# euroexa/spmv-fpga

Measured on AMD Instinct MI355X. Metric: SpMV GFLOP/s + effective HBM GB/s (% roofline), fp64, 1/2/4/8 MI355X, higher is better.
Workload: dtype f64

## Files before the change

spmv-fpga_amd/csrc/layout.cpp:

```cpp
#include <algorithm>
#include <cmath>

#include "spmv_host.hpp"

namespace spmvhw {

int plan_panels(const char *who, const IndexType *h_rp, IndexType n, uint64_t nnz, uint32_t rmax,
                const panel_options &o, panel_cut &out)
{
    const uint64_t wgs = o.wgs;
    std::vector<uint32_t> &prow = out.prow;
    double xbias = o.xbias;
    bool split_mode = false, subdivide = false;
    for (uint64_t P = o.P_first;; ++P) {
        {
            const uint64_t S = P ? wgs / P : 0;
            split_mode = !subdivide && o.allow_split && S >= 2 && P * S * 10 >= wgs * 9 &&
                         (o.force_split || 2 * S * n * o.acc_bytes * 5 <= 3 * nnz * (4 + o.val_bytes));
        }
        if (!split_mode && P > 1 && P % wgs)
            P = (P + wgs - 1) / wgs * wgs;
        P = std::min<uint64_t>(P, std::max<uint64_t>(n, 1));
        prow.assign(1, 0);
        bool ok = true;
        IndexType r = 0;
        for (uint64_t q = 1; q <= P && ok; ++q) {
            const uint64_t target =
                split_mode || xbias == 0.0
                    ? nnz * q / P
                    : (uint64_t)(double(nnz) * (double(q) - xbias * double(q & 1)) / (double(P) - xbias * double(P & 1)));
            IndexType e = (q == P) ? n : (IndexType)(std::lower_bound(h_rp, h_rp + n + 1, (IndexType)target) - h_rp);
            e = std::max(e, r);
            if (e - r > rmax && xbias != 0.0 && !split_mode && q < P)
                e = r + rmax;
            if (e - r > rmax && subdivide)
                for (; e - r > rmax; r += rmax)
                    prow.push_back(r + rmax);
            if (e - r > rmax)
                ok = false;
            prow.push_back(e);
            r = e;
        }
        if (ok)
            break;
        if (xbias != 0.0 && !split_mode) {
            xbias = 0.0;
            --P;
            continue;
        }
        if (P >= n || P > 8 * std::max<uint64_t>(min_panels(n, rmax), wgs)) {
            if (subdivide) {
                set_error(std::string(who) + ": cannot form panels");
                return 1;
            }
            subdivide = true;
            xbias = 0.0;
            P = o.P_first - 1;
        }
    }
    out.split_mode = split_mode;
    out.xbias = xbias;
    return 0;
}

static void cut_units(const std::vector<uint32_t> &poff, const std::vector<uint32_t> &punit, double d,
                      std::vector<uint32_t> &uent)
{
    const uint32_t P = (uint32_t)punit.size() - 1, U = punit[P];
    uent.assign((size_t)U + 1, 0);
    auto wc = [&](uint32_t u) { return double(u) - d * double(u & 1); };
    for (uint32_t q = 0; q < P; ++q) {
        const uint64_t chunks = (uint64_t(poff[q + 1]) - poff[q]) / kSweepChunk;
        const uint32_t k = punit[q + 1] - punit[q], u0 = punit[q];
        for (uint32_t t = 0; t < k; ++t) {
            const uint64_t c = d != 0.0 ? (uint64_t)(double(chunks) * (wc(u0 + t) - wc(u0)) / (wc(u0 + k) - wc(u0)))
                                        : chunks * t / k;
            uent[u0 + t] = (uint32_t)(poff[q] + kSweepChunk * c);
        }
    }
    uent[U] = poff[P];
}

int plan_sweep_units(const char *who, const IndexType *h_rp, const std::vector<uint32_t> &prow, bool split_mode,
                     uint64_t wgs, int pieces_override, double xbias_split, sweep_units &out)
{
    const uint32_t P = (uint32_t)(prow.size() - 1);
    std::vector<uint32_t> &off = out.off, &poff = out.poff, &punit = out.punit, &upanel = out.upanel;
    off.assign((size_t)P + 1, 0);
    poff.assign((size_t)P + 1, 0);
    out.rmax_used = 0;
    uint64_t padded = 0;
    for (uint32_t q = 0; q < P; ++q) {
        const uint64_t cnt = uint64_t(h_rp[prow[q + 1]]) - h_rp[prow[q]];
        padded += (cnt + kSweepChunk - 1) / kSweepChunk * kSweepChunk;
        off[q + 1] = (uint32_t)(off[q] + cnt);
        poff[q + 1] = (uint32_t)padded;
        out.rmax_used = std::max(out.rmax_used, prow[q + 1] - prow[q]);
    }
    if (padded > 0xFFFFFFFFull) {
        set_error(std::string(who) + ": padded entry count exceeds 32 bits");
        return 2;
    }
    uint32_t split = split_mode ? std::max<uint32_t>(1, (uint32_t)(wgs / P)) : 1;
    if (split_mode && pieces_override > 0)
        split = (uint32_t)pieces_override;
    const double mean = P ? double(padded) / P : 0.0;
    punit.assign((size_t)P + 1, 0);
    for (uint32_t q = 0; q < P; ++q) {
        const uint64_t chunks = (uint64_t(poff[q + 1]) - poff[q]) / kSweepChunk;
        uint64_t k = split * std::max<uint64_t>(
                                 1, (uint64_t)std::ceil(double(poff[q + 1] - poff[q]) / std::max(2.0 * mean, 1.0)));
        k = std::max<uint64_t>(1, std::min<uint64_t>(k, chunks));
        punit[q + 1] = punit[q] + (uint32_t)k;
    }
    upanel.assign(std::max<uint32_t>(punit[P], 1), 0);
    bool multi = false;
    for (uint32_t q = 0; q < P; ++q) {
        multi |= punit[q + 1] - punit[q] > 1;
        for (uint32_t u = punit[q]; u < punit[q + 1]; ++u)
            upanel[u] = q;
    }
    out.xbias_split = split_mode ? xbias_split : 0.0;
    cut_units(poff, punit, out.xbias_split, out.uent);
    out.sweep_split = multi ? std::max<uint32_t>(split, 2) : 1;
    return 0;
}

bin_windows plan_bin_windows(uint64_t ncols, uint64_t cus, double d)
{
    constexpr uint64_t PER = kBinPer;
    bin_windows w;
    const uint64_t wmax = w.wmax = std::min<uint64_t>((kSweepLdsBytes - 256) / sizeof(ValueType) / PER * PER, 65536);
    uint64_t &nwin = w.nwin, &W = w.W, &W0 = w.W0, &W1 = w.W1;
    if (ncols) {
        const uint64_t rounds = std::max<uint64_t>(1, (ncols + cus * wmax - 1) / (cus * wmax));
        nwin = std::min<uint64_t>(cus * rounds, (ncols + PER - 1) / PER);
        W = ((ncols + nwin - 1) / nwin + PER - 1) / PER * PER;
        nwin = (ncols + W - 1) / W;
    }
    W0 = W1 = W;
    if (!(d > -0.25 && d < 0.25) || nwin < cus || nwin % cus)
        d = 0.0;
    const uint64_t w0 = std::min<uint64_t>(wmax, (uint64_t(std::llround(W * (1.0 + d))) + PER / 2) / PER * PER);
    if (d != 0.0 && w0 >= PER && w0 < 2 * W) {
        W0 = w0;
        W1 = 2 * W - w0;
        if (W1 > wmax) {
            W0 = W1 = W;
        }
        const uint64_t pw = W0 + W1, k = ncols / pw, rem = ncols - k * pw;
        nwin = 2 * k + (rem == 0 ? 0 : rem <= W0 ? 1 : 2);
    }
    return w;
}

void plan_bin_units(const std::vector<uint32_t> &cnt, const std::vector<uint32_t> &esc, uint64_t nwin, uint64_t P,
                    uint64_t cus, bin_units &out)
{
    constexpr uint64_t PER = kBinPer;
    const uint64_t nseg = nwin * P;
    std::vector<uint64_t> &seg = out.seg, &ub = out.ub;
    seg.assign(nseg + 1, 0);
    for (uint64_t k = 0; k < nseg; ++k) {
        seg[k + 1] = seg[k] + (uint64_t(cnt[k]) + esc[k] + PER - 1) / PER * PER;
        if ((k + 1) % P == 0)
            seg[k + 1] = (seg[k + 1] + kBinAlign - 1) / kBinAlign * kBinAlign;
    }
    const uint64_t ent_pad = seg[nseg];
    ub.assign(1, 0);
    out.uwin.clear();
    const double mean = nwin ? double(ent_pad) / double(nwin) : 0.0;
    const uint64_t fill = nwin < cus ? (cus + nwin - 1) / nwin : 1;
    for (uint64_t w = 0; w < nwin; ++w) {
        const uint64_t a = seg[w * P], b = seg[(w + 1) * P], e = b - a;
        if (!e)
            continue;
        uint64_t k = std::max<uint64_t>(fill, (uint64_t)std::ceil(double(e) / std::max(2.0 * mean, 1.0)));
        k = std::max<uint64_t>(1, std::min<uint64_t>(k, e / kBinAlign));
        ub.back() = a;
        for (uint64_t t = 1; t <= k; ++t) {
            ub.push_back(a + (e / kBinAlign) * t / k * kBinAlign);
            out.uwin.push_back((uint32_t)w);
        }
    }
}

}
```

spmv-fpga_amd/csrc/plan.cpp:

```cpp
#include <algorithm>
#include <chrono>
#include <cstdlib>
#include <cstring>
#include <memory>
#include <mutex>
#include <thread>

#include "spmv_internal.hpp"

static int run_impl(spmv_plan *p, const ValueType *d_x, ValueType *d_y, hipStream_t s, bool timing);

namespace spmvhw {

int upload_staged(void *dst, const void *src, size_t bytes, hipStream_t s)
{
    constexpr size_t kChunk = 32u << 20;
    if (bytes < (4u << 20)) {
        SPMV_TRY(hipMemcpyAsync(dst, src, bytes, hipMemcpyHostToDevice, s));
        SPMV_TRY(hipStreamSynchronize(s));
        return 0;
    }
    static std::mutex mu;
    static void *buf[2] = {nullptr, nullptr};
    static hipEvent_t done[2] = {nullptr, nullptr};
    std::lock_guard<std::mutex> lk(mu);
    for (int i = 0; i < 2; ++i) {
        if (!buf[i])
            SPMV_TRY(hipHostMalloc(&buf[i], kChunk, hipHostMallocPortable));
        if (!done[i])
            SPMV_TRY(hipEventCreateWithFlags(&done[i], hipEventDisableTiming));
    }
    bool pending[2] = {false, false};
    const unsigned hc = std::thread::hardware_concurrency();
    const int T = (int)std::min(4u, hc ? hc : 1u);
    int i = 0;
    for (size_t off = 0; off < bytes; off += kChunk, i ^= 1) {
        const size_t n = std::min(kChunk, bytes - off);
        if (pending[i])
            SPMV_TRY(hipEventSynchronize(done[i]));
        auto part = [&](int t) {
            const size_t b = n * t / T, e = n * (t + 1) / T;
            std::memcpy((char *)buf[i] + b, (const char *)src + off + b, e - b);
        };
        std::vector<std::thread> th;
        for (int t = 1; t < T; ++t)
            th.emplace_back(part, t);
        part(0);
        for (auto &t : th)
            t.join();
        SPMV_TRY(hipMemcpyAsync((char *)dst + off, buf[i], n, hipMemcpyHostToDevice, s));
        SPMV_TRY(hipEventRecord(done[i], s));
        pending[i] = true;
    }
    SPMV_TRY(hipStreamSynchronize(s));
    return 0;
}

int slice_from_device(const char *who, csr_slice &out, const void *handle, int device, IndexType n, IndexType m,
                      IndexType nr_nzeros, const IndexType *d_row_ptr, const IndexType *d_col, const ValueType *d_val,
                      hipStream_t stream)
{
    if (slice_device_args(who, handle, n, d_row_ptr))
        return 1;
    SPMV_TRY(hipSetDevice(device));
    out.n = n;
    out.m = m;
    out.rp.assign(size_t(n) + 1, 0u);
    if (n) {
        SPMV_TRY(hipMemcpyAsync(out.rp.data(), d_row_ptr, out.rp.size() * sizeof(IndexType), hipMemcpyDeviceToHost,
                                stream));
        SPMV_TRY(hipStreamSynchronize(stream));
    }
    out.col = d_col;
    out.val = d_val;
    out.on_device = true;
    out.stream = stream;
    return slice_rebase(who, out, &nr_nzeros);
}

int slice_entries_on_device(const csr_slice &sl, device_scratch &up_col, device_scratch &up_val,
                            const IndexType **d_col, const ValueType **d_val)
{
    *d_col = sl.col;
    *d_val = sl.val;
    const uint64_t nnz = sl.nnz();
    if (sl.on_device || !nnz)
        return 0;
    hipStream_t s = (hipStream_t)sl.stream;
    SPMV_TRY(hipMalloc(&up_col.p, nnz * sizeof(IndexType)));
    SPMV_TRY(hipMalloc(&up_val.p, nnz * sizeof(ValueType)));
    if (upload_staged(up_col.p, sl.col, nnz * sizeof(IndexType), s) ||
        upload_staged(up_val.p, sl.val, nnz * sizeof(ValueType), s))
        return 1;
    *d_col = (const IndexType *)up_col.p;
    *d_val = (const ValueType *)up_val.p;
    return 0;
}

struct PhaseTrace {
    const bool on = std::getenv("SPMV_HW_TRACE") != nullptr;
    std::chrono::steady_clock::time_point t0 = std::chrono::steady_clock::now(), last = t0;
    void operator()(const char *phase, hipStream_t s)
    {
        if (!on)
            return;
        (void)hipStreamSynchronize(s);
        const auto now = std::chrono::steady_clock::now();
        std::fprintf(stderr, "spmv_hw trace: %-28s %9.3f ms (total %9.3f ms)\n", phase,
                     std::chrono::duration<double, std::milli>(now - last).count(),
                     std::chrono::duration<double, std::milli>(now - t0).count());
        last = now;
    }
};

constexpr int kKernelTune = -2;

static int requested_kernel()
{
    const char *e = std::getenv("SPMV_HW_KERNEL");
    if (!e || !*e || !std::strcmp(e, "auto"))
        return -1;
    if (!std::strcmp(e, "tune"))
        return kKernelTune;
    if (!std::strcmp(e, "tiles"))
        return kKernelTiles;
    if (!std::strcmp(e, "sweep"))
        return kKernelSweep;
    if (!std::strcmp(e, "gold"))
        return kKernelGold;
    if (!std::strcmp(e, "fpga"))
        return kKernelFpga;
    if (!std::strcmp(e, "blocked"))
        return kKernelBlocked;
    if (!std::strcmp(e, "slices"))
        return kKernelSlices;
    if (!std::strcmp(e, "binned"))
        return kKernelBinned;
    return -1;
}

static int build_gold(spmv_plan &p, const IndexType *h_row_ptr, const IndexType *d_col_src,
                      const ValueType *d_val_src, hipStream_t s)
{
    p.nlong = 0;
    for (IndexType r = 0; r < p.nr_rows; ++r)
        p.nlong += h_row_ptr[r + 1] - h_row_ptr[r] > (IndexType)kGoldLong;
    SPMV_TRY(hipMalloc((void **)&p.d_rp, (size_t(p.nr_rows) + 1) * sizeof(uint32_t)));
    SPMV_TRY(hipMalloc((void **)&p.d_col, std::max<uint64_t>(p.nnz, 1) * sizeof(uint32_t)));
    SPMV_TRY(hipMalloc((void **)&p.d_val, std::max<uint64_t>(p.nnz, 1) * sizeof(ValueType)));
    SPMV_TRY(hipMemcpyAsync(p.d_rp, h_row_ptr, (size_t(p.nr_rows) + 1) * sizeof(uint32_t), hipMemcpyHostToDevice, s));
    if (p.nnz) {
        SPMV_TRY(hipMemcpyAsync(p.d_col, d_col_src, p.nnz * sizeof(uint32_t), hipMemcpyDeviceToDevice, s));
        SPMV_TRY(hipMemcpyAsync(p.d_val, d_val_src, p.nnz * sizeof(ValueType), hipMemcpyDeviceToDevice, s));
    }
    SPMV_TRY(hipStreamSynchronize(s));
    return 0;
}

static int build_tiles(spmv_plan &p, const IndexType *h_row_ptr, const IndexType *d_col_src,
                       const ValueType *d_val_src, hipStream_t s)
{
    const IndexType nr_rows = p.nr_rows;
    const uint64_t nnz = p.nnz;
    p.nnz_pad = (nnz + kTileNnz - 1) / kTileNnz * kTileNnz;
    p.ntiles = p.nnz_pad / kTileNnz;

    std::vector<uint32_t> rowend(p.nnz_pad / 32, 0u);
    std::vector<uint32_t> row_id;
    if (p.has_empty)
        row_id.reserve(p.nzr);
    for (IndexType r = 0; r < nr_rows; ++r) {
        if (h_row_ptr[r + 1] > h_row_ptr[r]) {
            const uint64_t e = h_row_ptr[r + 1] - 1ull;
            rowend[e >> 5] |= 1u << (e & 31);
            if (p.has_empty)
                row_id.push_back(r);
        }
    }
    std::vector<uint32_t> tile_info(p.ntiles + 1, 0u);
    {
        uint64_t rr = 0, c = 0;
        for (uint64_t t = 0; t <= p.ntiles; ++t) {
            const uint64_t k = t * kTileNnz;
            while (rr < nr_rows && h_row_ptr[rr + 1] <= k) {
                if (h_row_ptr[rr + 1] > h_row_ptr[rr])
                    ++c;
                ++rr;
            }
            if (c > 0x7FFFFFFFull) {
                set_error("too many non-empty rows for the tile table");
                return 1;
            }
            const bool cont = k > 0 && k < nnz && !((rowend[(k - 1) >> 5] >> ((k - 1) & 31)) & 1u);
            tile_info[t] = (uint32_t)(c << 1) | (cont ? 1u : 0u);
        }
    }
    std::vector<uint32_t> cross;
    {
        auto bit = [&](uint64_t k) { return (rowend[k >> 5] >> (k & 31)) & 1u; };
        std::vector<uint8_t> has_tail(p.ntiles, 0), has_end(p.ntiles, 0);
        for (uint64_t t = 0; t < p.ntiles; ++t) {
            const uint64_t w0 = t * (kTileNnz / 32);
            for (uint64_t w = 0; w < kTileNnz / 32; ++w)
                has_end[t] |= rowend[w0 + w] != 0;
            const uint64_t last = (t + 1) * kTileNnz - 1;
            has_tail[t] = (last + 1 < nnz) && !bit(last);
        }
        for (uint64_t t = 0; t < p.ntiles; ++t) {
            if (!has_tail[t] || !(has_end[t] || t == 0 || !has_tail[t - 1]))
                continue;
            uint64_t j = t + 1;
            while (j < p.ntiles && !has_end[j])
                ++j;
            if (j >= p.ntiles) {
                set_error("internal: unterminated row crossing");
                return 1;
            }
            cross.push_back(tile_info[t + 1] >> 1);
            cross.push_back((uint32_t)t);
            cross.push_back((uint32_t)j);
        }
        p.ncross = cross.size() / 3;
    }
    auto alloc = [&](void **ptr, size_t bytes) -> hipError_t {
        *ptr = nullptr;
        return bytes ? hipMalloc(ptr, bytes) : hipSuccess;
    };
    SPMV_TRY(alloc((void **)&p.d_col, p.nnz_pad * sizeof(uint32_t)));
    SPMV_TRY(alloc((void **)&p.d_val, p.nnz_pad * sizeof(ValueType)));
    SPMV_TRY(alloc((void **)&p.d_rowend, rowend.size() * sizeof(uint32_t)));
    SPMV_TRY(alloc((void **)&p.d_tile_info, tile_info.size() * sizeof(uint32_t)));
    SPMV_TRY(alloc((void **)&p.d_head, p.ntiles * sizeof(ValueType)));
    SPMV_TRY(alloc((void **)&p.d_tail, p.ntiles * sizeof(ValueType)));
    SPMV_TRY(alloc((void **)&p.d_cross, cross.size() * sizeof(uint32_t)));
    if (p.has_empty)
        SPMV_TRY(alloc((void **)&p.d_row_id, row_id.size() * sizeof(uint32_t)));
    if (!rowend.empty())
        SPMV_TRY(hipMemcpyAsync(p.d_rowend, rowend.data(), rowend.size() * 4, hipMemcpyHostToDevice, s));
    SPMV_TRY(hipMemcpyAsync(p.d_tile_info, tile_info.data(), tile_info.size() * 4, hipMemcpyHostToDevice, s));
    if (p.has_empty && !row_id.empty())
        SPMV_TRY(hipMemcpyAsync(p.d_row_id, row_id.data(), row_id.size() * 4, hipMemcpyHostToDevice, s));
    if (!cross.empty())
        SPMV_TRY(hipMemcpyAsync(p.d_cross, cross.data(), cross.size() * 4, hipMemcpyHostToDevice, s));
    if (p.nnz_pad)
        SPMV_TRY(launch_pack(d_col_src, d_val_src, nnz, p.nnz_pad, p.nr_cols, p.d_col, p.d_val, nullptr, s));
    if (const char *xe = ablation_env("SPMV_TILE_XCD"))
        p.tile_xcd = xe[0] == '1';
    const char *nenv = ablation_env("SPMV_TILE_NARROW");
    const int narrow_min = !nenv || !*nenv ? 1 : std::atoi(nenv) == 16 ? 2 : std::atoi(nenv) == 0 ? 4 : 1;
    if (p.ntiles && narrow_min < 4) {
        uint32_t *d_span = nullptr;
        SPMV_TRY(alloc((void **)&p.d_tile_cbase, p.ntiles * sizeof(uint32_t)));
        SPMV_TRY(alloc((void **)&d_span, sizeof(uint32_t)));
        uint32_t span = 0xFFFFFFFFu;
        hipError_t e = hipMemsetAsync(d_span, 0, sizeof(uint32_t), s);
        if (e == hipSuccess)
            e = launch_tile_span(p.d_col, nnz, p.ntiles, p.d_tile_cbase, d_span, s);
        if (e == hipSuccess)
            e = hipMemcpyAsync(&span, d_span, sizeof(uint32_t), hipMemcpyDeviceToHost, s);
        if (e == hipSuccess)
            e = hipStreamSynchronize(s);
        (void)hipFree(d_span);
        SPMV_TRY(e);
        const int cb = span < 256u && narrow_min <= 1 ? 1 : span < 65536u ? 2 : 4;
        if (cb < 4) {
            SPMV_TRY(alloc(&p.d_colnar, p.nnz_pad * cb));
            SPMV_TRY(launch_narrow(p.d_col, nnz, p.nnz_pad, p.d_tile_cbase, p.d_colnar, cb, s));
            SPMV_TRY(hipStreamSynchronize(s));
            SPMV_TRY(hipFree(p.d_col));
            p.d_col = nullptr;
            p.tile_col_bytes = cb;
        } else {
            SPMV_TRY(hipFree(p.d_tile_cbase));
            p.d_tile_cbase = nullptr;
            const char *cenv = ablation_env("SPMV_TILE_CLUSTER");
            if (!(cenv && cenv[0] == '0')) {
                uint32_t *d_bad = nullptr;
                SPMV_TRY(alloc((void **)&p.d_tile_cbase, p.ntiles * 4 * sizeof(uint32_t)));
                SPMV_TRY(alloc((void **)&d_bad, sizeof(uint32_t)));
                uint32_t bad = 1;
                e = hipMemsetAsync(d_bad, 0, sizeof(uint32_t), s);
                if (e == hipSuccess)
                    e = launch_tile_clusters(p.d_col, nnz, p.ntiles, p.d_tile_cbase, d_bad, s);
                if (e == hipSuccess)
                    e = hipMemcpyAsync(&bad, d_bad, sizeof(uint32_t), hipMemcpyDeviceToHost, s);
                if (e == hipSuccess)
                    e = hipStreamSynchronize(s);
                (void)hipFree(d_bad);
                SPMV_TRY(e);
                if (!bad) {
                    SPMV_TRY(alloc(&p.d_colnar, p.nnz_pad * 2));
                    SPMV_TRY(launch_cluster_encode(p.d_col, nnz, p.nnz_pad, p.d_tile_cbase, (uint16_t *)p.d_colnar, s));
                    SPMV_TRY(hipStreamSynchronize(s));
                    SPMV_TRY(hipFree(p.d_col));
                    p.d_col = nullptr;
                    p.tile_col_bytes = 2;
                    p.tile_clustered = true;
                } else {
                    SPMV_TRY(hipFree(p.d_tile_cbase));
                    p.d_tile_cbase = nullptr;
                }
            }
        }
    }
    SPMV_TRY(hipStreamSynchronize(s));
    return 0;
}

static int fpga_params(spmv_plan &p)
{
    if (const char *v = std::getenv("SPMV_FPGA_VF")) {
        const int vf = std::atoi(v);
        if (vf != 1 && vf != 2 && vf != 4 && vf != 8) {
            set_error("SPMV_FPGA_VF must be 1, 2, 4 or 8");
            return 1;
        }
        p.fpga_vf = vf;
    }
    if (const char *b = std::getenv("SPMV_FPGA_BLOCK")) {
        const long w = std::atol(b);
        if (w < 1 || w > 0x7FFFFFFFL) {
            set_error("SPMV_FPGA_BLOCK must be a positive column count");
            return 1;
        }
        p.fpga_width = (uint32_t)w;
    }
    return 0;
}

static int order_rows_by_block(spmv_plan &p, const IndexType *h_row_ptr, hipStream_t s)
{
    if (fpga_params(p))
        return 1;
    if (!p.nnz)
        return 0;
    std::vector<uint32_t> col(p.nnz);
    SPMV_TRY(hipMemcpyAsync(col.data(), p.d_col, p.nnz * 4, hipMemcpyDeviceToHost, s));
    SPMV_TRY(hipStreamSynchronize(s));
    bool sorted = true;
    for (IndexType r = 0; r < p.nr_rows && sorted; ++r)
        for (uint64_t k = uint64_t(h_row_ptr[r]) + 1; k < h_row_ptr[r + 1]; ++k)
            if (col[k] / p.fpga_width < col[k - 1] / p.fpga_width) {
                sorted = false;
                break;
            }
    if (sorted)
        return 0;
    std::vector<ValueType> val(p.nnz);
    SPMV_TRY(hipMemcpyAsync(val.data(), p.d_val, p.nnz * sizeof(ValueType), hipMemcpyDeviceToHost, s));
    SPMV_TRY(hipStreamSynchronize(s));
    std::vector<uint32_t> idx;
    std::vector<uint32_t> c2(col);
    std::vector<ValueType> v2(val);
    for (IndexType r = 0; r < p.nr_rows; ++r) {
        const uint64_t b = h_row_ptr[r], e = h_row_ptr[r + 1];
        idx.resize(e - b);
        for (uint64_t k = b; k < e; ++k)
            idx[k - b] = (uint32_t)k;
        std::stable_sort(idx.begin(), idx.end(),
                         [&](uint32_t i, uint32_t j) { return col[i] / p.fpga_width < col[j] / p.fpga_width; });
        for (uint64_t k = b; k < e; ++k) {
            c2[k] = col[idx[k - b]];
            v2[k] = val[idx[k - b]];
        }
    }
    SPMV_TRY(hipMemcpyAsync(p.d_col, c2.data(), p.nnz * 4, hipMemcpyHostToDevice, s));
    SPMV_TRY(hipMemcpyAsync(p.d_val, v2.data(), p.nnz * sizeof(ValueType), hipMemcpyHostToDevice, s));
    SPMV_TRY(hipStreamSynchronize(s));
    return 0;
}

static int build_layout(spmv_plan &P, int kernel, bool automatic, const IndexType *h_row_ptr,
                        const IndexType *d_col, const ValueType *d_val, hipStream_t s)
{
    P.kernel = kernel;
    if (kernel == kKernelBinned) {
        const int rc = build_binned(P, h_row_ptr, d_col, d_val, s);
        if (rc == 2 && automatic) {
            P.kernel = kernel = kKernelSweep;
            (void)hipGetLastError();
        } else if (rc) {
            return 1;
        }
    }
    if (kernel == kKernelSweep || kernel == kKernelSlices) {
        const int rc = kernel == kKernelSweep ? build_sweep(P, h_row_ptr, d_col, d_val, s)
                                              : build_slices(P, h_row_ptr, d_col, d_val, s);
        if (rc == 2 && automatic)
            P.kernel = kernel = kKernelTiles;
        else if (rc)
            return 1;
    }
    if (kernel == kKernelSweep || kernel == kKernelSlices || kernel == kKernelBinned) {
    } else if (kernel == kKernelBlocked) {
        if (fpga_params(P) || build_blocked(P, h_row_ptr, d_col, d_val, s))
            return 1;
    } else if (kernel == kKernelGold || kernel == kKernelFpga) {
        if (build_gold(P, h_row_ptr, d_col, d_val, s))
            return 1;
        if (kernel == kKernelFpga && order_rows_by_block(P, h_row_ptr, s))
            return 1;
    } else {
        if (build_tiles(P, h_row_ptr, d_col, d_val, s))
            return 1;
    }
    SPMV_TRY(hipStreamSynchronize(s));
    if (P.kernel == kKernelSweep) {
        (void)launch_sweep(P, nullptr, nullptr, s, true);
    } else if (P.kernel == kKernelBinned) {
        (void)launch_binned(P, nullptr, nullptr, s, true);
    } else if (P.kernel == kKernelBlocked) {
        (void)launch_blocked(P, nullptr, nullptr, s, true);
    } else if (P.kernel == kKernelSlices) {
        (void)launch_slices(P, nullptr, nullptr, s, true);
    } else if (P.kernel == kKernelGold || P.kernel == kKernelFpga) {
        (void)launch_gold(P, nullptr, nullptr, s, true);
    } else {
        (void)launch_spmv(P, nullptr, nullptr, s, true);
        (void)launch_fixup(P, nullptr, s, true);
    }
    (void)hipGetLastError();
    return 0;
}

constexpr int kTuneSteps = 4, kTuneReps = 7;
static int time_layout(spmv_plan &P, const ValueType *d_x, ValueType *d_y, hipStream_t s, double *ms)
{
    SPMV_TRY(hipStreamSynchronize(s));
    struct Res {
        hipStream_t ts = nullptr;
        hipGraphExec_t ge = nullptr;
        hipEvent_t ev[2 * kTuneReps] = {};
        ~Res()
        {
            for (hipEvent_t e : ev)
                if (e)
                    (void)hipEventDestroy(e);
            if (ge)
                (void)hipGraphExecDestroy(ge);
            if (ts)
                (void)hipStreamDestroy(ts);
        }
    } r;
    SPMV_TRY(hipStreamCreateWithFlags(&r.ts, hipStreamNonBlocking));
    for (hipEvent_t &e : r.ev)
        SPMV_TRY(hipEventCreate(&e));
    SPMV_TRY(hipStreamBeginCapture(r.ts, hipStreamCaptureModeRelaxed));
    int rc = 0;
    for (int i = 0; i < kTuneSteps && !rc; ++i)
        rc = ::run_impl(&P, d_x, d_y, r.ts, false);
    hipGraph_t g = nullptr;
    const hipError_t ec = hipStreamEndCapture(r.ts, &g);
    if (rc) {
        if (g)
            (void)hipGraphDestroy(g);
        return rc;
    }
    SPMV_TRY(ec);
    const hipError_t ei = hipGraphInstantiate(&r.ge, g, nullptr, nullptr, 0);
    (void)hipGraphDestroy(g);
    SPMV_TRY(ei);
    SPMV_TRY(hipGraphLaunch(r.ge, r.ts));
    for (int k = 0; k < kTuneReps; ++k) {
        SPMV_TRY(hipEventRecord(r.ev[2 * k], r.ts));
        SPMV_TRY(hipGraphLaunch(r.ge, r.ts));
        SPMV_TRY(hipEventRecord(r.ev[2 * k + 1], r.ts));
    }
    SPMV_TRY(hipStreamSynchronize(r.ts));
    std::vector<double> t(kTuneReps);
    for (int k = 0; k < kTuneReps; ++k) {
        float v = 0.f;
        SPMV_TRY(hipEventElapsedTime(&v, r.ev[2 * k], r.ev[2 * k + 1]));
        t[k] = v / kTuneSteps;
    }
    std::nth_element(t.begin(), t.begin() + kTuneReps / 2, t.end());
    *ms = t[kTuneReps / 2];
    return 0;
}

int plan_create_from_slice(spmv_plan **out, int device, int op, const csr_slice &sl, int force_kernel)
{
    *out = nullptr;
    if (op == SPMV_OP_T) {
        SPMV_TRY(hipSetDevice(device));
        transposed_csr t;
        if (transpose_slice(t, sl) || plan_create_from_slice(out, device, SPMV_OP_N, t.slice, force_kernel))
            return 1;
        (*out)->op = SPMV_OP_T;
        return 0;
    }
    PhaseTrace trace;
    const IndexType nr_rows = sl.n, nr_cols = sl.m;
    const IndexType *h_row_ptr = sl.rp.data();
    hipStream_t s = (hipStream_t)sl.stream;
    const uint64_t nnz = sl.nnz();
    uint64_t nzr = 0;
    for (IndexType r = 0; r < nr_rows; ++r)
        nzr += h_row_ptr[r + 1] > h_row_ptr[r];
    if (nnz > 0 && nr_cols == 0) {
        set_error("matrix has non-zeros but zero columns");
        return 1;
    }
    SPMV_TRY(hipSetDevice(device));

    std::unique_ptr<spmv_plan> p(new spmv_plan());
    p->device = device;
    p->nr_rows = nr_rows;
    p->nr_cols = nr_cols;
    p->nnz = nnz;
    p->nzr = nzr;
    p->has_empty = nzr < nr_rows;

    device_scratch tcol, tval, trp, tbad;
    const IndexType *d_col = nullptr;
    const ValueType *d_val = nullptr;
    if (slice_entries_on_device(sl, tcol, tval, &d_col, &d_val))
        return 1;
    trace("row_ptr scan + upload", s);
    if (nnz) {
        SPMV_TRY(hipMalloc(&tbad.p, sizeof(uint32_t)));
        SPMV_TRY(hipMemsetAsync(tbad.p, 0, sizeof(uint32_t), s));
        SPMV_TRY(launch_validate(d_col, nnz, nr_cols, (uint32_t *)tbad.p, s));
        uint32_t bad = 0;
        SPMV_TRY(hipMemcpyAsync(&bad, tbad.p, sizeof(bad), hipMemcpyDeviceToHost, s));
        SPMV_TRY(hipStreamSynchronize(s));
        if (bad) {
            set_error("column index out of range (>= nr_cols)");
            return 1;
        }
    }

    const int requested = force_kernel >= 0 ? force_kernel : requested_kernel();
    int kernel = requested;
    const bool tune = kernel == kKernelTune;
    if (kernel == -1 || tune) {
        kernel = kKernelTiles;
        if (nnz && uint64_t(nr_cols) * sizeof(ValueType) >= (2ull << 20) && nnz >= 16ull * kSweepThreads) {
            SPMV_TRY(hipMalloc(&trp.p, (size_t(nr_rows) + 1) * sizeof(IndexType)));
            SPMV_TRY(hipMemcpyAsync(trp.p, h_row_ptr, (size_t(nr_rows) + 1) * sizeof(IndexType),
                                    hipMemcpyHostToDevice, s));
            if (probe_locality((const IndexType *)trp.p, d_col, nr_rows, s, &p->locality))
                return 1;
            if (p->locality < 0.3)
                kernel = kKernelSweep;
        }
        const char *det = std::getenv("SPMV_SWEEP_DETERMINISTIC");
        if (kernel == kKernelSweep && sizeof(ValueType) == 4 && nr_cols >= 5000000u && nnz >= 16000000ull &&
            !(det && det[0] == '1'))
            kernel = kKernelBinned;
    }
    const int auto_kernel = kernel;
    if (tune)
        kernel = kKernelTune;
    trace("validate + kernel choice", s);
    if (const char *t = ablation_env("SPMV_SWEEP_THREADS")) {
        const int v = std::atoi(t);
        if (v == 256 || v == 512 || v == 1024)
            p->sweep_threads = v;
    }
    auto fresh = [&]() {
        std::unique_ptr<spmv_plan> q(new spmv_plan());
        q->device = p->device;
        q->nr_rows = p->nr_rows;
        q->nr_cols = p->nr_cols;
        q->nnz = p->nnz;
        q->nzr = p->nzr;
        q->has_empty = p->has_empty;
        q->sweep_threads = p->sweep_threads;
        q->locality = p->locality;
        return q;
    };
    if (kernel == kKernelTune) {
        const char *det = std::getenv("SPMV_SWEEP_DETERMINISTIC");
        const bool fixed_bits = det && det[0] == '1';
        constexpr double kTuneBand = 0.97;
        device_scratch tx, ty;
        SPMV_TRY(hipMalloc(&tx.p, std::max<size_t>(nr_cols, 1) * sizeof(ValueType)));
        SPMV_TRY(hipMalloc(&ty.p, std::max<size_t>(nr_rows, 1) * sizeof(ValueType)));
        SPMV_TRY(hipMemsetAsync(tx.p, 0, std::max<size_t>(nr_cols, 1) * sizeof(ValueType), s));
        const int slot_of[7] = {0, -1, 1, -1, -1, 2, 3};
        std::vector<int> order = {auto_kernel};
        for (int k : {kKernelTiles, kKernelSweep, kKernelSlices, kKernelBinned})
            if (k != auto_kernel)
                order.push_back(k);
        double tuned[4] = {1e30, 1e30, 1e30, 1e30};
        std::unique_ptr<spmv_plan> kept;
        double kept_ms = 1e30;
        for (int k : order) {
            if (k == kKernelBinned && fixed_bits)
                continue;
            std::unique_ptr<spmv_plan> q = fresh();
            if (k == kKernelSlices)
                q->slice_pad_limit = 2.0;
            double t = 1e30;
            if (build_layout(*q, k, true, h_row_ptr, d_col, d_val, s) ||
                time_layout(*q, (const ValueType *)tx.p, (ValueType *)ty.p, s, &t)) {
                q.reset();
                (void)hipGetLastError();
                continue;
            }
            tuned[slot_of[k]] = t;
            if (!kept || t < kTuneBand * kept_ms) {
                kept.swap(q);
                kept_ms = t;
            }
        }
        if (!kept) {
            if (build_layout(*p, kKernelTiles, true, h_row_ptr, d_col, d_val, s))
                return 1;
        } else {
            p.swap(kept);
        }
        if (std::getenv("SPMV_HW_TRACE"))
            std::fprintf(stderr, "spmv_hw trace: tune ms tiles %.4f sweep %.4f slices %.4f binned %.4f -> kernel %d\n",
                         tuned[0], tuned[1], tuned[2], tuned[3], p->kernel);
        for (int c = 0; c < 4; ++c)
            p->tuned_ms[c] = tuned[c];
        trace("tune: build + time each", s);
    } else if (requested < 0 && kernel == kKernelTiles && nnz >= 65536) {
        std::unique_ptr<spmv_plan> r = fresh();
        r->slice_pad_limit = 1.15;
        const int rc = build_layout(*r, kKernelSlices, true, h_row_ptr, d_col, d_val, s);
        if (rc == 0 && r->kernel == kKernelSlices &&
            (r->slice_off_bytes == 2 || (r->slice_off_bytes == 1 && sizeof(ValueType) == 4)) &&
            double(r->slice_slots) * kWave <= 1.15 * double(nnz)) {
            p.swap(r);
            trace("build slice layout", s);
        } else if (rc == 0 && r->kernel == kKernelTiles) {
            r->slice_pad_limit = 0.0;
            p.swap(r);
            trace("build tile layout", s);
        } else {
            r.reset();
            (void)hipGetLastError();
            if (build_layout(*p, kKernelTiles, true, h_row_ptr, d_col, d_val, s))
                return 1;
            trace("build tile layout", s);
        }
    } else {
        if (kernel == kKernelBinned && requested < 0) {
            p->bin_skew_limit = 2.0;
            p->bin_row_limit = 0.3;
            if (const char *e = std::getenv("SPMV_BIN_ROW_LIMIT"))
                p->bin_row_limit = std::atof(e);
        }
        if (build_layout(*p, kernel, requested < 0, h_row_ptr, d_col, d_val, s))
            return 1;
        trace(p->kernel == kKernelSweep ? "build sweep layout" : p->kernel == kKernelBinned ? "build binned layout"
              : p->kernel != kKernelTiles ? "build CSR layout"
                                                                                        : "build tile layout", s);
    }
    *out = p.release();
    return 0;
}

bool product_variant(int kernel, int variant)
{
    if (variant == 0)
        return true;
    if (kernel == kKernelSweep)
        return variant == 28 || variant == kSweepTurnOrdered;
    if (kernel == kKernelBinned)
        return variant == 1 || variant == 2;
    return false;
}

}

using namespace spmvhw;

spmv_plan::~spmv_plan()
{
    (void)hipSetDevice(device);
    (void)hipDeviceSynchronize();
    for (void *ptr : {(void *)d_col, (void *)d_val, (void *)d_rowend, (void *)d_tile_info,
                      (void *)d_row_id, (void *)d_head, (void *)d_tail, (void *)d_cross, (void *)d_s_col,
                      (void *)d_s_row, (void *)d_s_val, (void *)d_panel_row, (void *)d_unit_ent, (void *)d_part, (void *)d_gcount, (void *)d_steal, (void *)d_panel_cnt, (void *)d_unit_panel, (void *)d_panel_unit, (void *)d_rp,
                      (void *)d_s_cbase, (void *)d_s_row16, (void *)d_s_d8, (void *)d_s_dbase, (void *)d_s_side, d_colnar, (void *)d_tile_cbase, (void *)d_kptr, (void *)d_kpos,
                      (void *)d_rp2, (void *)d_rl, (void *)d_chunk_row, (void *)d_bpart, (void *)d_slot_off,
                      (void *)d_sbase, (void *)d_slice_len, (void *)d_b_val, (void *)d_b_colw, (void *)d_b_rowp,
                      d_b_prod_alloc, (void *)d_b_seg, (void *)d_b_seg_hi, (void *)d_b_ub, (void *)d_b_uwin})
        if (ptr)
            (void)hipFree(ptr);
    for (void *ptr : gpart)
        (void)hipFree(ptr);
    for (hipEvent_t e : ev)
        (void)hipEventDestroy(e);
    if (gexec)
        (void)hipGraphExecDestroy(gexec);
    if (gstream)
        (void)hipStreamDestroy(gstream);
    if (gstream2)
        (void)hipStreamDestroy(gstream2);
}

uint64_t spmv_plan::device_bytes() const
{
    if (kernel == kKernelGold || kernel == kKernelFpga)
        return (uint64_t(nr_rows) + 1) * 4 + nnz * (4 + sizeof(ValueType));
    if (kernel == kKernelSlices)
        return slice_slots * kWave * (sizeof(ValueType) + slice_off_bytes) + slice_slots * (slice_clustered ? 16 : 4) +
               (nslices + 1) * 4 +
               uint64_t(nr_rows) * 4;
    if (kernel == kKernelBlocked)
        return nnz * (2 + sizeof(ValueType)) + (nkpairs + 1) * 4 + nkpairs * (4 + 2 + sizeof(ValueType)) +
               (uint64_t(nr_rows) + 1) * 4 + (nchunks + 1) * 4 + nunits * 8 + 4;
    if (kernel == kKernelBinned)
        return ent_pad * (2 * sizeof(ValueType) + 2 + (b_delta ? 1 : 2)) + (uint64_t(b_nwin) * npanels + 1) * 8 +
               (b_nunits + 1) * 12 + (npanels + 1) * 4;
    if (kernel == kKernelSweep)
        return ent_pad * ((d_s_col ? sizeof(uint32_t) : 0) + (sweep_packed ? 0 : sizeof(uint16_t)) + sizeof(ValueType)) +
               (npanels + 1) * 4 + (nunits + 1) * 4 + (sweep_packed ? ent_pad / kSweepChunk * 4 : 0) +
               (sweep_split > 1 ? nunits * (uint64_t(panel_rmax) + 1) * sweep_acc_bytes : 0) + nunits * 4 + (npanels + 1) * 4 +
               (d_panel_cnt ? npanels * 4 : 0) +
               (sweep_delta ? ent_pad * 3 + ent_pad / kSweepChunk * 4 + sweep_side_chunks * kSweepChunk * 4 : 0);
    return nnz_pad * (tile_col_bytes + sizeof(ValueType)) + nnz_pad / 8 + (ntiles + 1) * 4 +
           (tile_col_bytes < 4 ? ntiles * (tile_clustered ? 16 : 4) : 0) +
           (has_empty ? nzr * 4 : 0) + ntiles * 2 * sizeof(ValueType) + ncross * 12;
}

uint64_t spmv_plan::algorithmic_bytes() const
{
    return nnz * (sizeof(ValueType) + 4) + (uint64_t(nr_rows) + 1) * 4 +
           uint64_t(nr_cols) * sizeof(ValueType) + uint64_t(nr_rows) * sizeof(ValueType);
}

static int create_device(const char *who, spmv_plan **plan, int device, int op, IndexType nr_rows, IndexType nr_cols,
                         IndexType nr_nzeros, const IndexType *d_row_ptr, const IndexType *d_col_ind,
                         const ValueType *d_values, void *stream)
{
    csr_slice sl;
    if (slice_from_device(who, sl, plan, device, nr_rows, nr_cols, nr_nzeros, d_row_ptr, d_col_ind, d_values,
                          (hipStream_t)stream))
        return 1;
    return plan_create_from_slice(plan, device, op, sl);
}

static int create_host(const char *who, spmv_plan **plan, int device, int op, const csr_matrix *m, IndexType row_begin,
                       IndexType row_end)
{
    csr_slice sl;
    if (slice_from_host(who, sl, plan, m, row_begin, row_end))
        return 1;
    return plan_create_from_slice(plan, device, op, sl);
}

extern "C" {

int spmv_plan_create_device(spmv_plan **plan, int device, IndexType nr_rows, IndexType nr_cols,
                            IndexType nr_nzeros, const IndexType *d_row_ptr,
                            const IndexType *d_col_ind, const ValueType *d_values, void *stream)
{
    return create_device("spmv_plan_create_device", plan, device, SPMV_OP_N, nr_rows, nr_cols, nr_nzeros, d_row_ptr,
                         d_col_ind, d_values, stream);
}

int spmv_plan_create_host(spmv_plan **plan, int device, const csr_matrix *m, IndexType row_begin,
                          IndexType row_end)
{
    return create_host("spmv_plan_create_host", plan, device, SPMV_OP_N, m, row_begin, row_end);
}

int spmv_plan_create_device_op(spmv_plan **plan, int device, int op, IndexType nr_rows, IndexType nr_cols,
                               IndexType nr_nzeros, const IndexType *d_row_ptr, const IndexType *d_col_ind,
                               const ValueType *d_values, void *stream)
{
    if (bad_op("spmv_plan_create_device_op", op))
        return 1;
    return create_device(op == SPMV_OP_N ? "spmv_plan_create_device" : "spmv_plan_create_device_op", plan, device, op,
                         nr_rows, nr_cols, nr_nzeros, d_row_ptr, d_col_ind, d_values, stream);
}

int spmv_plan_create_host_op(spmv_plan **plan, int device, int op, const csr_matrix *m, IndexType row_begin,
                             IndexType row_end)
{
    if (bad_op("spmv_plan_create_host_op", op))
        return 1;
    return create_host(op == SPMV_OP_N ? "spmv_plan_create_host" : "spmv_plan_create_host_op", plan, device, op, m,
                       row_begin, row_end);
}

int spmv_plan_get_op(const spmv_plan *plan, int *op)
{
    if (!plan || !op) {
        set_error("spmv_plan_get_op: null argument");
        return 1;
    }
    *op = plan->op;
    return 0;
}

static int run_impl(spmv_plan *p, const ValueType *d_x, ValueType *d_y, hipStream_t s, bool timing)
{
    if (p->nr_rows == 0)
        return 0;
    if (p->kernel == kKernelTiles && (p->has_empty || p->nnz == 0))
        SPMV_TRY(hipMemsetAsync(d_y, 0, size_t(p->nr_rows) * sizeof(ValueType), s));
    hipEvent_t e0 = nullptr, e1 = nullptr;
    if (timing) {
        if (p->ev_used + 2 > p->ev.size()) {
            for (int i = 0; i < 2; ++i) {
                hipEvent_t e;
                SPMV_TRY(hipEventCreate(&e));
                p->ev.push_back(e);
            }
        }
        e0 = p->ev[p->ev_used];
        e1 = p->ev[p->ev_used + 1];
        p->ev_used += 2;
        SPMV_TRY(hipEventRecord(e0, s));
    }
    if (p->kernel != kKernelTiles) {
        SPMV_TRY(p->kernel == kKernelSweep     ? launch_sweep(*p, d_x, d_y, s)
                 : p->kernel == kKernelBinned  ? launch_binned(*p, d_x, d_y, s)
                 : p->kernel == kKernelBlocked ? launch_blocked(*p, d_x, d_y, s)
                 : p->kernel == kKernelSlices  ? launch_slices(*p, d_x, d_y, s)
                                               : launch_gold(*p, d_x, d_y, s));
        if (timing)
            SPMV_TRY(hipEventRecord(e1, s));
        return 0;
    }
    SPMV_TRY(launch_spmv(*p, d_x, d_y, s));
    if (timing)
        SPMV_TRY(hipEventRecord(e1, s));
    SPMV_TRY(launch_fixup(*p, d_y, s));
    return 0;
}

int spmv_plan_run(const spmv_plan *cp, const ValueType *d_x, ValueType *d_y, void *stream)
{
    if (!cp) {
        set_error("spmv_plan_run: null plan");
        return 1;
    }
    spmv_plan *p = const_cast<spmv_plan *>(cp);
    SPMV_TRY(hipSetDevice(p->device));
    return run_impl(p, d_x, d_y, (hipStream_t)stream, p->timing);
}

static bool graph_overlaps(const spmv_plan *p)
{
    return p->kernel == kKernelSweep && p->sweep_split > 1 && !p->d_panel_cnt && p->d_part &&
           !(p->sweep_variant >= 37 && p->sweep_variant <= 39);
}

static int graph_part2(spmv_plan *p)
{
    if (p->gpart.empty()) {
        void *b = nullptr;
        SPMV_TRY(hipMalloc(&b, p->nunits * (uint64_t(p->panel_rmax) + 1) * p->sweep_acc_bytes));
        p->gpart.push_back(b);
    }
    return 0;
}

static int capture_overlapped(spmv_plan *p, const ValueType *d_x, ValueType *d_y, int iters)
{
    constexpr int R = 2;
    if (graph_part2(p))
        return 1;
    if (!p->gstream2)
        SPMV_TRY(hipStreamCreateWithFlags(&p->gstream2, hipStreamNonBlocking));
    std::vector<hipEvent_t> ev(2 * size_t(iters), nullptr);
    auto destroy = [&] {
        for (hipEvent_t e : ev)
            if (e)
                (void)hipEventDestroy(e);
    };
    for (auto &e : ev)
        if (hipEventCreateWithFlags(&e, hipEventDisableTiming) != hipSuccess) {
            destroy();
            set_error("spmv_plan_run_graph: hipEventCreate failed");
            return 1;
        }
    hipStream_t a = p->gstream, b = p->gstream2;
    hipError_t e = hipStreamBeginCapture(a, hipStreamCaptureModeRelaxed);
    for (int k = 0; k < iters && e == hipSuccess; ++k) {
        void *part = k % R ? p->gpart[k % R - 1] : p->d_part;
        if (k >= R)
            e = hipStreamWaitEvent(a, ev[2 * (k - R) + 1], 0);
        if (e == hipSuccess)
            e = launch_sweep(*p, d_x, d_y, a, false, 1, part);
        if (e == hipSuccess)
            e = hipEventRecord(ev[2 * k], a);
        if (e == hipSuccess)
            e = hipStreamWaitEvent(b, ev[2 * k], 0);
        if (e == hipSuccess)
            e = launch_sweep(*p, d_x, d_y, b, false, 2, part);
        if (e == hipSuccess)
            e = hipEventRecord(ev[2 * k + 1], b);
    }
    if (e == hipSuccess)
        e = hipStreamWaitEvent(a, ev[2 * (iters - 1) + 1], 0);
    hipGraph_t g = nullptr;
    const hipError_t ec = hipStreamEndCapture(a, &g);
    destroy();
    if (e != hipSuccess || ec != hipSuccess) {
        if (g)
            (void)hipGraphDestroy(g);
        set_error(std::string("spmv_plan_run_graph: overlapped capture: ") +
                  hipGetErrorString(e != hipSuccess ? e : ec));
        return 1;
    }
    const hipError_t ei = hipGraphInstantiate(&p->gexec, g, nullptr, nullptr, 0);
    (void)hipGraphDestroy(g);
    SPMV_TRY(ei);
    return 0;
}

static int capture_behind(spmv_plan *p, const ValueType *d_x, ValueType *d_y, int iters)
{
    if (graph_part2(p))
        return 1;
    if (!p->d_gcount) {
        SPMV_TRY(hipMalloc(&p->d_gcount, 2 * sizeof(uint32_t)));
        SPMV_TRY(hipMemset(p->d_gcount, 0, 2 * sizeof(uint32_t)));
    }
    int ncu = 0;
    SPMV_TRY(hipDeviceGetAttribute(&ncu, hipDeviceAttributeMultiprocessorCount, p->device));
    auto part_of = [&](int k) { return (k & 1) ? p->gpart[0] : p->d_part; };
    hipStream_t a = p->gstream;
    hipError_t e = hipStreamBeginCapture(a, hipStreamCaptureModeRelaxed);
    for (int k = 0; k < iters && e == hipSuccess; ++k) {
        sweep_behind bh;
        bh.cpart = k ? part_of(k - 1) : nullptr;
        bh.ccount = p->d_gcount + (k & 1);
        bh.cnext = p->d_gcount + ((k + 1) & 1);
        bh.blocks = (uint32_t)std::max(ncu, 1);
        if (const char *v = ablation_env("SPMV_BEHIND_BLOCKS"))
            bh.blocks = (uint32_t)std::max(1, atoi(v));
        if (const char *v = ablation_env("SPMV_BEHIND_ROWS"))
            bh.rows_per_thread = (uint32_t)std::max(1, atoi(v) / std::max(1, p->sweep_threads));
        e = launch_sweep(*p, d_x, d_y, a, false, 1, part_of(k), &bh);
    }
    if (e == hipSuccess)
        e = launch_sweep(*p, d_x, d_y, a, false, 2, part_of(iters - 1));
    hipGraph_t g = nullptr;
    const hipError_t ec = hipStreamEndCapture(a, &g);
    if (e != hipSuccess || ec != hipSuccess) {
        if (g)
            (void)hipGraphDestroy(g);
        set_error(std::string("spmv_plan_run_graph: behind capture: ") + hipGetErrorString(e != hipSuccess ? e : ec));
        return 1;
    }
    const hipError_t ei = hipGraphInstantiate(&p->gexec, g, nullptr, nullptr, 0);
    (void)hipGraphDestroy(g);
    SPMV_TRY(ei);
    return 0;
}

static int graph_form(const spmv_plan *p)
{
    const int best = p->kernel == kKernelSweep && sweep_behind_ok(*p) ? 2 : graph_overlaps(p) ? 1 : 0;
    if (const char *f = ablation_env("SPMV_GRAPH_FORM")) {
        const std::string v(f);
        if (v == "serial")
            return 0;
        if (v == "dag" && best >= 1)
            return 1;
    }
    return best;
}

int spmv_plan_run_graph(spmv_plan *p, const ValueType *d_x, ValueType *d_y, int iters, void *stream)
{
    if (!p || iters < 1) {
        set_error("spmv_plan_run_graph: null plan or iters < 1");
        return 1;
    }
    hipStream_t s = (hipStream_t)stream;
    SPMV_TRY(hipSetDevice(p->device));
    if (!p->gexec || p->gx != d_x || p->gy != d_y || p->giters != iters) {
        if (p->gexec) {
            SPMV_TRY(hipGraphExecDestroy(p->gexec));
            p->gexec = nullptr;
        }
        if (!p->gstream)
            SPMV_TRY(hipStreamCreateWithFlags(&p->gstream, hipStreamNonBlocking));
        const int form = iters >= 2 ? graph_form(p) : 0;
        if (form == 2) {
            if (capture_behind(p, d_x, d_y, iters))
                return 1;
        } else if (form == 1) {
            if (capture_overlapped(p, d_x, d_y, iters))
                return 1;
        } else {
            SPMV_TRY(hipStreamBeginCapture(p->gstream, hipStreamCaptureModeRelaxed));
            int rc = 0;
            for (int i = 0; i < iters && !rc; ++i)
                rc = run_impl(p, d_x, d_y, p->gstream, false);
            hipGraph_t g = nullptr;
            const hipError_t ec = hipStreamEndCapture(p->gstream, &g);
            if (rc) {
                if (g)
                    (void)hipGraphDestroy(g);
                return rc;
            }
            SPMV_TRY(ec);
            const hipError_t ei = hipGraphInstantiate(&p->gexec, g, nullptr, nullptr, 0);
            (void)hipGraphDestroy(g);
            SPMV_TRY(ei);
        }
        p->gx = d_x;
        p->gy = d_y;
        p->giters = iters;
    }
    hipEvent_t e0 = nullptr, e1 = nullptr;
    if (p->timing) {
        for (int i = 0; p->ev_used + 2 > p->ev.size() && i < 2; ++i) {
            hipEvent_t e;
            SPMV_TRY(hipEventCreate(&e));
            p->ev.push_back(e);
        }
        e0 = p->ev[p->ev_used];
        e1 = p->ev[p->ev_used + 1];
        p->ev_used += 2;
        SPMV_TRY(hipEventRecord(e0, s));
    }
    SPMV_TRY(hipGraphLaunch(p->gexec, s));
    if (p->timing)
        SPMV_TRY(hipEventRecord(e1, s));
    return 0;
}

int spmv_plan_get_stats(const spmv_plan *p, spmv_plan_stats *st)
{
    if (!p || !st) {
        set_error("spmv_plan_get_stats: null argument");
        return 1;
    }
    std::memset(st, 0, sizeof(*st));
    st->nr_rows = p->nr_rows;
    st->nr_cols = p->nr_cols;
    st->nr_nzeros = p->nnz;
    st->nr_nonempty_rows = p->nzr;
    const bool csr = p->kernel == kKernelGold || p->kernel == kKernelFpga;
    st->nr_tiles = (p->kernel == kKernelSweep || p->kernel == kKernelBlocked) ? p->nunits
                   : p->kernel == kKernelBinned                               ? p->npanels
                   : p->kernel == kKernelSlices                               ? p->nslices
                   : csr                                                      ? p->nlong
                                                                              : p->ntiles;
    st->tile_nnz = p->kernel == kKernelSlices   ? p->slice_slots * kWave
                   : p->kernel == kKernelSweep  ? (p->nunits ? p->ent_pad / p->nunits : 0)
                   : p->kernel == kKernelBinned ? (p->npanels ? p->ent_pad / p->npanels : 0)
                   : p->kernel == kKernelBlocked ? (p->nunits ? p->nnz / p->nunits : 0)
                   : csr                         ? (uint64_t)kGoldLong
                                                 : kTileNnz;
    st->device_bytes = p->device_bytes();
    st->algorithmic_bytes = p->algorithmic_bytes();
    st->device = p->device;
    st->kernel = p->kernel;
    st->blocks = p->kernel == kKernelBlocked ? (uint32_t)((uint64_t(p->nr_cols) + p->fpga_width - 1) / p->fpga_width) : 1;
    st->format = (p->kernel == kKernelSlices && p->slice_off_bytes < 4 ? 1 : 0) | (p->slice_clustered ? 16 : 0) |
                 (p->kernel == kKernelSlices && p->slice_off_bytes == 1 ? 8 : 0) | (p->tile_col_bytes < 4 ? 1 : 0) | (p->sweep_packed ? 2 : 0) | (p->sweep_lane_order ? 4 : 0) | (p->sweep_delta ? 64 : 0) |
                 (p->tile_col_bytes == 1 ? 8 : 0) | (p->tile_clustered ? 16 : 0) |
                 (p->kernel == kKernelBinned && p->b_delta ? 32 : 0) |
                 (p->kernel == kKernelSweep && p->sweep_steal &&
                          (p->sweep_variant == 37 || p->sweep_variant == 38 || p->sweep_variant == 39) ? 128 : 0) |
                 (graph_form(p) == 2 ? 256 : graph_form(p) == 1 ? 512 : 0) |
                 (p->kernel == kKernelSweep && p->sweep_split > 1 && p->xbias_split > 0.0 ? 1024 : 0) |
                 (p->kernel == kKernelSweep && p->sweep_split > 1 && p->xbias_split < 0.0 ? 2048 : 0) |
                 (p->kernel == kKernelSweep && p->sweep_wide ? 4096 : 0);
    return 0;
}

int spmv_plan_set_variant(spmv_plan *p, int variant)
{
    if (!p || variant < 0 || (variant > 63 && variant != kSweepTurn && variant != kSweepTurnOrdered)) {
        set_error("spmv_plan_set_variant: bad arguments");
        return 1;
    }
#ifndef SPMV_ABLATIONS
    if (!product_variant(p->kernel, variant)) {
        set_error("spmv_plan_set_variant: measurement variant (tools library only)");
        return 1;
    }
#endif
    if (p->kernel == kKernelSweep && variant == 0)
        variant = 28;
    if (p->kernel == kKernelSweep) {
        if ((variant < 36 || variant > 39) && variant != 28 && sweep_materialize_rc(*p))
            return 1;
        p->sweep_variant = variant;
    } else if (p->kernel == kKernelBinned) {
        if (variant > 7 && !(variant >= 51 && variant <= 52)) {
            set_error("spmv_plan_set_variant: binned variants are 0-7");
            return 1;
        }
        if (p->d_b_seg_hi) {
            SPMV_TRY(hipSetDevice(p->device));
            SPMV_TRY(hipFree(p->d_b_seg_hi));
            p->d_b_seg_hi = nullptr;
            p->b_seg_base = 0;
        }
        if (variant == 1 || variant == 2) {
            SPMV_TRY(hipSetDevice(p->device));
            const uint64_t nseg = uint64_t(p->b_nwin) * p->npanels + 1;
            std::vector<uint64_t> h(nseg);
            SPMV_TRY(hipMemcpy(h.data(), p->d_b_seg, nseg * 8, hipMemcpyDeviceToHost));
            const uint64_t base = (variant == 1 ? (1ull << 31) : (1ull << 32)) - h[nseg - 1] / 2;
            for (auto &v : h)
                v += base;
            SPMV_TRY(hipMalloc((void **)&p->d_b_seg_hi, nseg * 8));
            SPMV_TRY(hipMemcpy(p->d_b_seg_hi, h.data(), nseg * 8, hipMemcpyHostToDevice));
            p->b_seg_base = base;
        }
        p->variant = variant;
    } else {
        p->variant = variant & 3;
    }
    if (p->gexec) {
        (void)hipSetDevice(p->device);
        (void)hipGraphExecDestroy(p->gexec);
        p->gexec = nullptr;
    }
    return 0;
}

int spmv_plan_set_timing(spmv_plan *p, int enable)
{
    if (!p) {
        set_error("spmv_plan_set_timing: null plan");
        return 1;
    }
    p->timing = enable != 0;
    p->ev_used = 0;
    return 0;
}

int spmv_plan_get_timing(spmv_plan *p, double *mean_ms, double *total_ms, int *launches)
{
    if (!p) {
        set_error("spmv_plan_get_timing: null plan");
        return 1;
    }
    SPMV_TRY(hipSetDevice(p->device));
    double tot = 0.0;
    int n = 0;
    for (size_t i = 0; i + 1 < p->ev_used; i += 2) {
        SPMV_TRY(hipEventSynchronize(p->ev[i + 1]));
        float ms = 0.f;
        SPMV_TRY(hipEventElapsedTime(&ms, p->ev[i], p->ev[i + 1]));
        tot += ms;
        ++n;
    }
    p->ev_used = 0;
    if (mean_ms)
        *mean_ms = n ? tot / n : 0.0;
    if (total_ms)
        *total_ms = tot;
    if (launches)
        *launches = n;
    return 0;
}

void spmv_plan_destroy(spmv_plan *p) { delete p; }

}
```

spmv-fpga_amd/csrc/spmv_host.hpp:

```cpp
#pragma once

#include <algorithm>
#include <cstddef>
#include <cstdint>
#include <cstdlib>
#include <string>
#include <vector>

#include "csr_hw_wrapper.h"

namespace spmvhw {

void set_error(const std::string &msg);
const char *get_error();

inline const char *ablation_env(const char *name)
{
#ifdef SPMV_ABLATIONS
    return std::getenv(name);
#else
    (void)name;
    return nullptr;
#endif
}

struct csr_slice {
    IndexType n = 0, m = 0;
    std::vector<IndexType> rp;
    const IndexType *col = nullptr;
    const ValueType *val = nullptr;
    bool on_device = false;
    void *stream = nullptr;
    uint64_t nnz() const { return rp.empty() ? 0 : rp.back(); }
};

int slice_from_host(const char *who, csr_slice &out, const void *handle, const csr_matrix *m, IndexType row_begin,
                    IndexType row_end);
int slice_device_args(const char *who, const void *handle, IndexType n, const IndexType *d_row_ptr);
int slice_rebase(const char *who, csr_slice &s, const IndexType *nr_nzeros = nullptr);

constexpr uint64_t kSweepLdsBytes = 160 * 1024;
constexpr uint64_t kSweepChunk = 128;
constexpr uint32_t kBinPer = 16 / sizeof(ValueType);
constexpr uint64_t kBinAlign = 128;

inline uint64_t min_panels(uint64_t n, uint32_t rmax) { return std::max<uint64_t>(1, (n + rmax - 1) / rmax); }

struct panel_options {
    uint64_t wgs = 256;
    uint64_t P_first = 1;
    bool allow_split = false;
    bool force_split = false;
    uint64_t acc_bytes = 8, val_bytes = sizeof(ValueType);
    double xbias = 0.0;
};
struct panel_cut {
    std::vector<uint32_t> prow;
    bool split_mode = false;
    double xbias = 0.0;
};
int plan_panels(const char *who, const IndexType *h_rp, IndexType n, uint64_t nnz, uint32_t rmax,
                const panel_options &o, panel_cut &out);

struct sweep_units {
    std::vector<uint32_t> off, poff;
    std::vector<uint32_t> punit;
    std::vector<uint32_t> upanel;
    std::vector<uint32_t> uent;
    uint32_t rmax_used = 0;
    uint32_t sweep_split = 1;
    double xbias_split = 0.0;
};
int plan_sweep_units(const char *who, const IndexType *h_rp, const std::vector<uint32_t> &prow, bool split_mode,
                     uint64_t wgs, int pieces_override, double xbias_split, sweep_units &out);

struct bin_windows {
    uint64_t wmax = 0, nwin = 1, W = kBinPer, W0 = kBinPer, W1 = kBinPer;
};
bin_windows plan_bin_windows(uint64_t ncols, uint64_t cus, double d);

struct bin_units {
    std::vector<uint64_t> seg;
    std::vector<uint64_t> ub;
    std::vector<uint32_t> uwin;
};
void plan_bin_units(const std::vector<uint32_t> &cnt, const std::vector<uint32_t> &esc, uint64_t nwin, uint64_t P,
                    uint64_t cus, bin_units &out);

double timestamp_us();

struct add_part {
    ValueType *dst;
    const ValueType *src;
    uint64_t count;
    void *ready;
};

struct accum_options {
    bool prefault = true;
    bool split = true;
    int threads = 16;
};

double host_accumulate(const add_part *parts, size_t nparts, int (*wait)(void *ready, std::string *err),
                       const accum_options &opts, bool *failed, std::string *err);

void prefault(ValueType *p, uint64_t count);

}
```

spmv-fpga_amd/csrc/spmv_internal.hpp:

```cpp
#pragma once

#include <hip/hip_runtime.h>
#include <cstdint>
#include <cstdio>
#include <string>
#include <vector>

#include "csr_hw_wrapper.h"
#include "spmv_host.hpp"

namespace spmvhw {

constexpr int kWave = 64;
constexpr int kLaneEntries = 4;
constexpr int kStep = kWave * kLaneEntries;
constexpr int kTileSteps = 2;
constexpr int kTileNnz = kStep * kTileSteps;
constexpr int kBlockThreads = 256;
constexpr int kSweepThreads = 1024;
constexpr int kSweepTurn = 91;
constexpr int kSweepTurnOrdered = 94;

constexpr int kKernelTiles = 0;
constexpr int kKernelGold = 1;
constexpr int kKernelSweep = 2;
constexpr int kKernelFpga = 3;
constexpr int kKernelBlocked = 4;
constexpr int kKernelSlices = 5;
constexpr int kKernelBinned = 6;
constexpr int kGoldLong = 128;

__device__ __forceinline__ uint32_t wave_inclusive_sum(uint32_t v0)
{
    uint32_t v = v0;
    v += __builtin_amdgcn_update_dpp(0u, v0, 0x111, 0xf, 0xf, true);
    v += __builtin_amdgcn_update_dpp(0u, v0, 0x112, 0xf, 0xf, true);
    v += __builtin_amdgcn_update_dpp(0u, v0, 0x113, 0xf, 0xf, true);
    v += __builtin_amdgcn_update_dpp(0u, v, 0x114, 0xf, 0xe, true);
    v += __builtin_amdgcn_update_dpp(0u, v, 0x118, 0xf, 0xc, true);
    v += __builtin_amdgcn_update_dpp(0u, v, 0x142, 0xa, 0xf, false);
    v += __builtin_amdgcn_update_dpp(0u, v, 0x143, 0xc, 0xf, false);
    return v;
}

}

struct spmv_plan {
    int device = 0;
    IndexType nr_rows = 0, nr_cols = 0;
    uint64_t nnz = 0, nnz_pad = 0;
    uint64_t nzr = 0;
    uint64_t ntiles = 0;
    bool has_empty = false;
    int kernel = 0;
    int op = SPMV_OP_N;
    int variant = 0;
    int sweep_variant = 28;

    uint32_t *d_col = nullptr;
    void *d_colnar = nullptr;
    uint32_t *d_tile_cbase = nullptr;
    int tile_col_bytes = 4;
    bool tile_clustered = false;
    bool tile_xcd = false;
    ValueType *d_val = nullptr;
    uint32_t *d_rowend = nullptr;
    uint32_t *d_tile_info = nullptr;
    uint32_t *d_row_id = nullptr;
    ValueType *d_head = nullptr;
    ValueType *d_tail = nullptr;
    uint32_t *d_cross = nullptr;
    uint64_t ncross = 0;

    uint32_t *d_rp = nullptr;
    uint64_t nlong = 0;
    int fpga_vf = 1;
    uint32_t fpga_width = 32768;

    uint32_t *d_kptr = nullptr;
    uint32_t *d_kpos = nullptr;
    uint32_t *d_rp2 = nullptr;
    uint16_t *d_rl = nullptr;
    uint32_t *d_chunk_row = nullptr;
    ValueType *d_bpart = nullptr;
    uint64_t nkpairs = 0, nchunks = 0;
    bool blocked_xlds = false;

    uint32_t *d_slot_off = nullptr;
    uint32_t *d_sbase = nullptr;
    uint32_t *d_slice_len = nullptr;
    uint64_t nslices = 0, slice_slots = 0;
    int slice_off_bytes = 4;
    bool slice_clustered = false;
    bool slice_acc_native = false;
    double slice_pad_limit = 0.0;

    uint64_t npanels = 0, ent_pad = 0;
    uint64_t nunits = 0;
    uint32_t sweep_split = 1;
    uint32_t *d_unit_panel = nullptr;
    uint32_t *d_panel_unit = nullptr;
    void *d_part = nullptr;
    std::vector<void *> gpart;
    uint32_t *d_gcount = nullptr;
    double xbias_split = 0.0;
    unsigned long long *d_steal = nullptr;
    bool sweep_steal = false;
    uint32_t *d_panel_cnt = nullptr;
    int sweep_acc_bytes = 8;
    uint32_t panel_rmax = 0;
    int sweep_threads = spmvhw::kSweepThreads;
    uint32_t *d_s_col = nullptr;
    uint16_t *d_s_row = nullptr;
    ValueType *d_s_val = nullptr;
    uint32_t *d_panel_row = nullptr;
    uint32_t *d_unit_ent = nullptr;
    uint32_t *d_s_cbase = nullptr;
    bool sweep_packed = false;
    bool sweep_lane_order = false;
    bool sweep_det = false;
    uint16_t *d_s_row16 = nullptr;
    uint8_t *d_s_d8 = nullptr;
    uint32_t *d_s_dbase = nullptr;
    uint32_t *d_s_side = nullptr;
    uint64_t sweep_side_chunks = 0;
    bool sweep_delta = false;
    bool sweep_wide = false;
    uint32_t b_nwin = 0, b_W = 0;
    uint32_t b_W1 = 0;
    uint64_t b_nunits = 0;
    ValueType *d_b_val = nullptr;
    uint16_t *d_b_colw = nullptr;
    void *d_b_rowp = nullptr;
    bool b_delta = false;
    bool b_prod_temporal = false;
    ValueType *d_b_prod = nullptr;
    void *d_b_prod_alloc = nullptr;
    uint64_t *d_b_seg = nullptr;
    uint64_t *d_b_seg_hi = nullptr;
    uint64_t b_seg_base = 0;
    uint64_t *d_b_ub = nullptr;
    uint32_t *d_b_uwin = nullptr;
    double bin_skew_limit = 0.0;
    double bin_row_limit = 0.0;
    uint32_t *y_flag = nullptr;
    uint32_t y_epoch = 0;
    ValueType *y_host = nullptr;
    double locality = -1.0;
    double tuned_ms[4] = {-1.0, -1.0, -1.0, -1.0};

    bool timing = false;
    std::vector<hipEvent_t> ev;
    size_t ev_used = 0;

    hipGraphExec_t gexec = nullptr;
    hipStream_t gstream = nullptr;
    hipStream_t gstream2 = nullptr;
    const ValueType *gx = nullptr;
    ValueType *gy = nullptr;
    int giters = 0;

    uint64_t device_bytes() const;
    uint64_t algorithmic_bytes() const;
    ~spmv_plan();
};

namespace spmvhw {

template <typename K, typename... Args>
inline void launch_or_warm(bool warm, K kernel, dim3 grid, dim3 block, size_t lds, hipStream_t s, Args... args)
{
    if (warm) {
        hipFuncAttributes a;
        (void)hipFuncGetAttributes(&a, reinterpret_cast<const void *>(kernel));
    } else {
        hipLaunchKernelGGL(kernel, grid, block, lds, s, args...);
    }
}

hipError_t launch_spmv(const spmv_plan &p, const ValueType *d_x, ValueType *d_y, hipStream_t s, bool warm = false);
hipError_t launch_fixup(const spmv_plan &p, ValueType *d_y, hipStream_t s, bool warm = false);
hipError_t launch_pack(const IndexType *d_col_src, const ValueType *d_val_src, uint64_t nnz,
                       uint64_t nnz_pad, uint32_t ncols, uint32_t *d_col, ValueType *d_val,
                       uint32_t *d_bad, hipStream_t s);
hipError_t launch_validate(const IndexType *d_col, uint64_t nnz, uint32_t ncols, uint32_t *d_bad, hipStream_t s);
hipError_t launch_tile_span(const uint32_t *d_col, uint64_t nnz, uint64_t ntiles, uint32_t *d_cbase,
                            uint32_t *d_maxspan, hipStream_t s);
hipError_t launch_tile_clusters(const uint32_t *d_col, uint64_t nnz, uint64_t ntiles, uint32_t *d_bases,
                                uint32_t *d_bad, hipStream_t s);
hipError_t launch_cluster_encode(const uint32_t *d_col, uint64_t nnz, uint64_t nnz_pad, const uint32_t *d_bases,
                                 uint16_t *d_out, hipStream_t s);
hipError_t launch_narrow(const uint32_t *d_col, uint64_t nnz, uint64_t nnz_pad, const uint32_t *d_cbase,
                         void *d_out, int bytes, hipStream_t s);

hipError_t launch_gold(const spmv_plan &p, const ValueType *d_x, ValueType *d_y, hipStream_t s, bool warm = false);

hipError_t launch_blocked(const spmv_plan &p, const ValueType *d_x, ValueType *d_y, hipStream_t s, bool warm = false);
int build_blocked(spmv_plan &p, const IndexType *h_rp, const IndexType *d_col_src, const ValueType *d_val_src,
                  hipStream_t s);

hipError_t launch_slices(const spmv_plan &p, const ValueType *d_x, ValueType *d_y, hipStream_t s, bool warm = false);
int build_slices(spmv_plan &p, const IndexType *h_rp, const IndexType *d_col_src, const ValueType *d_val_src,
                 hipStream_t s);
hipError_t launch_slices_multi(const spmv_plan &p, int nvec, const ValueType *d_X, ValueType *d_Y, hipStream_t s,
                               bool warm = false);

hipError_t launch_binned(const spmv_plan &p, const ValueType *d_x, ValueType *d_y, hipStream_t s, bool warm = false);
int build_binned(spmv_plan &p, const IndexType *h_rp, const IndexType *d_col_src, const ValueType *d_val_src,
                 hipStream_t s);

struct sweep_behind {
    const void *cpart = nullptr;
    uint32_t *ccount = nullptr;
    uint32_t *cnext = nullptr;
    uint32_t blocks = 0;
    uint32_t rows_per_thread = 4;
};
hipError_t launch_sweep(const spmv_plan &p, const ValueType *d_x, ValueType *d_y, hipStream_t s, bool warm = false,
                        int phase = 0, void *part = nullptr, const sweep_behind *behind = nullptr);
bool sweep_behind_ok(const spmv_plan &p);
bool product_variant(int kernel, int variant);
int build_sweep(spmv_plan &p, const IndexType *h_rp, const IndexType *d_col_src, const ValueType *d_val_src,
                hipStream_t s);
int probe_locality(const IndexType *d_rp, const IndexType *d_col, IndexType n, hipStream_t s, double *frac);
int sweep_materialize_rc(spmv_plan &p);
bool sweep_can_flag_panels(const spmv_plan &p);

struct device_scratch {
    void *p = nullptr;
    ~device_scratch()
    {
        if (p)
            (void)hipFree(p);
    }
};
template <typename T>
struct device_buf : device_scratch {
    device_buf() = default;
    device_buf(const device_buf &) = delete;
    T *get() const { return static_cast<T *>(p); }
    operator T *() const { return get(); }
    hipError_t alloc(uint64_t count) { return hipMalloc(&p, count * sizeof(T)); }
    hipError_t release()
    {
        void *q = p;
        p = nullptr;
        return q ? hipFree(q) : hipSuccess;
    }
    void swap(T *&owned)
    {
        T *q = get();
        p = owned;
        owned = q;
    }
};
template <typename K, typename... Args>
inline hipError_t launch_items(K kernel, uint64_t items, unsigned block, hipStream_t s, Args... args)
{
    hipLaunchKernelGGL(kernel, dim3((unsigned)((items + block - 1) / block)), dim3(block), 0, s, args...);
    return hipGetLastError();
}
inline int device_cu_count(int device)
{
    hipDeviceProp_t prop;
    return hipGetDeviceProperties(&prop, device) == hipSuccess && prop.multiProcessorCount > 0
               ? prop.multiProcessorCount
               : 256;
}

int upload_staged(void *dst, const void *src, size_t bytes, hipStream_t s);
int slice_from_device(const char *who, csr_slice &out, const void *handle, int device, IndexType n, IndexType m,
                      IndexType nr_nzeros, const IndexType *d_row_ptr, const IndexType *d_col, const ValueType *d_val,
                      hipStream_t stream);
int slice_entries_on_device(const csr_slice &sl, device_scratch &up_col, device_scratch &up_val,
                            const IndexType **d_col, const ValueType **d_val);
int plan_create_from_slice(spmv_plan **out, int device, int op, const csr_slice &sl, int force_kernel = -1);

bool bad_op(const char *who, int op);
int check_transpose_size(const char *who, uint64_t nnz);
int csr_transpose_device(IndexType n, IndexType m, const IndexType *h_rp, const IndexType *d_col,
                         const ValueType *d_val, IndexType *d_t_rp, IndexType *d_t_col, ValueType *d_t_val,
                         hipStream_t s);
struct transposed_csr {
    csr_slice slice;
    device_scratch col, val;
};
int transpose_slice(transposed_csr &t, const csr_slice &sl);

int mgpu_create_borrowed(spmv_mgpu **out, int n, const int *devices, const IndexType *bounds, IndexType nr_cols,
                         const spmv_plan *const *plans);
int mgpu_run_on(spmv_mgpu *mg, int exchange, const ValueType *const *x_dev);
const ValueType *mgpu_root_y(const spmv_mgpu *mg);
int mgpu_rccl_calls(const spmv_mgpu *mg);
}

#define SPMV_TRY(expr)                                                                        \
    do {                                                                                      \
        hipError_t e_ = (expr);                                                               \
        if (e_ != hipSuccess) {                                                               \
            spmvhw::set_error(std::string(#expr) + ": " + hipGetErrorString(e_));             \
            return 1;                                                                         \
        }                                                                                     \
    } while (0)
#define SPMV_BUILD_TRY(expr)                                                                          \
    do {                                                                                              \
        hipError_t e_ = (expr);                                                                       \
        if (e_ != hipSuccess) {                                                                       \
            spmvhw::set_error(std::string(kWho) + ": " + #expr + ": " + hipGetErrorString(e_));       \
            return 1;                                                                                 \
        }                                                                                             \
    } while (0)
```

spmv-fpga_amd/csrc/sweep.hip:

```cpp
#include <hipcub/hipcub.hpp>

#include <algorithm>
#include <tuple>
#include <cmath>
#include <cstring>

#include "spmv_internal.hpp"

namespace spmvhw {

__device__ __forceinline__ void lds_add(double *p, double v) { atomicAdd(p, v); }
__device__ __forceinline__ void lds_add(float *p, float v)
{
    uint32_t *u = reinterpret_cast<uint32_t *>(p);
    uint32_t old = *u, assumed;
    do {
        assumed = old;
        old = atomicCAS(u, assumed, __float_as_uint(__uint_as_float(assumed) + v));
    } while (old != assumed);
}

template <int N>
__device__ __forceinline__ void lds_add_n(double *y, const uint32_t (&idx)[N], const double (&v)[N])
{
#pragma unroll
    for (int i = 0; i < N; ++i)
        atomicAdd(&y[idx[i]], v[i]);
}
template <int N>
__device__ __forceinline__ void lds_add_n(float *y, const uint32_t (&idx)[N], const float (&v)[N])
{
    uint32_t *u = reinterpret_cast<uint32_t *>(y);
    uint32_t old[N], got[N];
#pragma unroll
    for (int i = 0; i < N; ++i)
        old[i] = __hip_atomic_load(&u[idx[i]], __ATOMIC_RELAXED, __HIP_MEMORY_SCOPE_WORKGROUP);
#pragma unroll
    for (int i = 0; i < N; ++i)
        got[i] = atomicCAS(&u[idx[i]], old[i], __float_as_uint(__uint_as_float(old[i]) + v[i]));
#pragma unroll
    for (int i = 0; i < N; ++i) {
        while (got[i] != old[i]) {
            old[i] = got[i];
            got[i] = atomicCAS(&u[idx[i]], old[i], __float_as_uint(__uint_as_float(old[i]) + v[i]));
        }
    }
}

typedef uint32_t u32x4 __attribute__((ext_vector_type(4)));
typedef uint16_t u16x4 __attribute__((ext_vector_type(4)));
typedef double f64x2 __attribute__((ext_vector_type(2)));
typedef float f32x4 __attribute__((ext_vector_type(4)));

template <bool NT, typename T>
__device__ __forceinline__ T lds_(const T *p)
{
    if constexpr (NT)
        return __builtin_nontemporal_load(p);
    else
        return *p;
}

template <bool NT>
__device__ __forceinline__ void load4(const double *__restrict__ v, uint64_t e, double (&o)[4])
{
    const f64x2 a = lds_<NT>(reinterpret_cast<const f64x2 *>(v + e));
    const f64x2 b = lds_<NT>(reinterpret_cast<const f64x2 *>(v + e + 2));
    o[0] = a.x; o[1] = a.y; o[2] = b.x; o[3] = b.y;
}
template <bool NT>
__device__ __forceinline__ void load4(const float *__restrict__ v, uint64_t e, float (&o)[4])
{
    const f32x4 a = lds_<NT>(reinterpret_cast<const f32x4 *>(v + e));
    o[0] = a.x; o[1] = a.y; o[2] = a.z; o[3] = a.w;
}

template <int E> struct EntryVec;
template <> struct EntryVec<4> { typedef u32x4 C; typedef u16x4 R; };
template <> struct EntryVec<1> {
    typedef uint32_t C __attribute__((ext_vector_type(1)));
    typedef uint16_t R __attribute__((ext_vector_type(1)));
};
template <> struct EntryVec<2> {
    typedef uint32_t C __attribute__((ext_vector_type(2)));
    typedef uint16_t R __attribute__((ext_vector_type(2)));
};

template <bool NT, int E, typename V>
__device__ __forceinline__ void loadv(const V *__restrict__ v, uint64_t e, V (&o)[E])
{
    if constexpr (E == 4) {
        load4<NT>(v, e, o);
    } else if constexpr (E == 1) {
        o[0] = lds_<NT>(v + e);
    } else if constexpr (sizeof(V) == 8) {
        const f64x2 a = lds_<NT>(reinterpret_cast<const f64x2 *>(v + e));
        o[0] = a.x; o[1] = a.y;
    } else {
        typedef float f32x2 __attribute__((ext_vector_type(2)));
        const f32x2 a = lds_<NT>(reinterpret_cast<const f32x2 *>(v + e));
        o[0] = a.x; o[1] = a.y;
    }
}

template <typename V, int T, typename A>
__device__ __forceinline__ void write_panel(const A *__restrict__ ylds, uint32_t R, V *__restrict__ y,
                                            uint32_t pieces, A *__restrict__ part, uint32_t stride,
                                            uint32_t u0, uint32_t *__restrict__ pcnt)
{
    if (pieces == 1) {
        for (uint32_t i = threadIdx.x; i < R; i += T)
            y[i] = V(ylds[i]);
        return;
    }
    A *dst = part + (uint64_t)blockIdx.x * stride;
    for (uint32_t i = threadIdx.x; i < R; i += T)
        dst[i] = ylds[i];
    if (!pcnt)
        return;
    __shared__ uint32_t last;
    asm volatile("s_waitcnt vmcnt(0)" ::: "memory");
    __syncthreads();
    if (threadIdx.x == 0) {
        __builtin_amdgcn_fence(__ATOMIC_RELEASE, "agent");
        asm volatile("s_waitcnt vmcnt(0)" ::: "memory");
        last = __hip_atomic_fetch_add(pcnt, 1u, __ATOMIC_RELAXED, __HIP_MEMORY_SCOPE_AGENT) == pieces - 1;
        if (last) {
            __builtin_amdgcn_fence(__ATOMIC_ACQUIRE, "agent");
            asm volatile("s_waitcnt vmcnt(0)" ::: "memory");
        }
    }
    __syncthreads();
    if (!last)
        return;
    const A *src = part + (uint64_t)u0 * stride;
    for (uint32_t i = threadIdx.x; i < R; i += T) {
        A acc = src[i];
        for (uint32_t t = 1; t < pieces; ++t)
            acc += src[(uint64_t)t * stride + i];
        y[i] = V(acc);
    }
    if (threadIdx.x == 0)
        __hip_atomic_store(pcnt, 0u, __ATOMIC_RELAXED, __HIP_MEMORY_SCOPE_AGENT);
}

template <typename V, typename A>
__global__ __launch_bounds__(256) void k_sweep_combine(const uint32_t *__restrict__ panel_row,
                                                       const uint32_t *__restrict__ panel_unit,
                                                       const A *__restrict__ part, uint32_t stride,
                                                       V *__restrict__ y, unsigned long long *__restrict__ steal)
{
    const uint32_t p = blockIdx.y;
    const uint32_t u0 = panel_unit[p], u1 = panel_unit[p + 1];
    if (steal && blockIdx.x == 0)
        for (uint32_t t = threadIdx.x; t < u1 - u0; t += 256)
            steal[u0 + t] = 0;
    const uint32_t r0 = panel_row[p], R = panel_row[p + 1] - r0;
    const uint32_t i = blockIdx.x * 256 + threadIdx.x;
    if (u1 - u0 < 2 || i >= R)
        return;
    const A *src = part + (uint64_t)u0 * stride + i;
    A acc = src[0];
    for (uint32_t t = 1; t < u1 - u0; ++t)
        acc += src[(uint64_t)t * stride];
    y[r0 + i] = V(acc);
}

template <typename V, int T, int E, int Q, bool SYNC, bool NT, typename A = double>
__global__ __launch_bounds__(T) void k_spmv_sweep(
    const uint32_t *__restrict__ col, const uint16_t *__restrict__ row, const V *__restrict__ val,
    const uint32_t *__restrict__ panel_row, const uint32_t *__restrict__ unit_ent,
    const uint32_t *__restrict__ unit_panel, const uint32_t *__restrict__ panel_unit,
    A *__restrict__ part, uint32_t stride, uint32_t *__restrict__ pcnt, const V *__restrict__ x,
    V *__restrict__ y)
{
    typedef typename EntryVec<E>::C CV;
    typedef typename EntryVec<E>::R RV;
    extern __shared__ __attribute__((aligned(16))) unsigned char smem[];
    A *ylds = reinterpret_cast<A *>(smem);
    const uint32_t p = unit_panel[blockIdx.x];
    const uint32_t pieces = panel_unit[p + 1] - panel_unit[p];
    const uint32_t r0 = panel_row[p], R = panel_row[p + 1] - r0;
    const uint64_t e0 = unit_ent[blockIdx.x], e1 = unit_ent[blockIdx.x + 1];
    for (uint32_t i = threadIdx.x; i <= R; i += T)
        ylds[i] = A(0);
    __syncthreads();
    constexpr uint64_t kGroup = (uint64_t)E * T;
    const uint64_t elast = e1 > e0 ? e1 - E : e0;
    for (uint64_t base = e0; base < e1; base += Q * kGroup) {
        CV c[Q];
        RV r[Q];
        V v[Q][E];
        bool ok[Q];
#pragma unroll
        for (int q = 0; q < Q; ++q) {
            uint64_t e = base + q * kGroup + (uint64_t)E * threadIdx.x;
            ok[q] = e < e1;
            e = ok[q] ? e : elast;
            c[q] = lds_<NT>(reinterpret_cast<const CV *>(col + e));
            r[q] = lds_<NT>(reinterpret_cast<const RV *>(row + e));
            loadv<NT, E>(val, e, v[q]);
        }
        V xv[Q][E];
#pragma unroll
        for (int q = 0; q < Q; ++q)
#pragma unroll
            for (int j = 0; j < E; ++j)
                xv[q][j] = x[c[q][j]];
#pragma unroll
        for (int q = 0; q < Q; ++q)
#pragma unroll
            for (int j = 0; j < E; ++j)
                lds_add(&ylds[ok[q] ? (uint32_t)r[q][j] : R], A(v[q][j]) * A(xv[q][j]));
        if constexpr (SYNC)
            __syncthreads();
    }
    __syncthreads();
    write_panel<V, T, A>(ylds, R, y + r0, pieces, part, stride, panel_unit[p], pcnt ? pcnt + p : nullptr);
}

#ifdef SPMV_ABLATIONS
__device__ unsigned long long g_abl_wg[4 * 4096];
#define ABL_WG_STAMP(k)                                                                            \
    do {                                                                                           \
        if (threadIdx.x == 0 && blockIdx.x < 4096)                                                 \
            g_abl_wg[4 * blockIdx.x + (k)] = __builtin_amdgcn_s_memrealtime();                     \
    } while (0)
#define ABL_WG_IDS()                                                                               \
    do {                                                                                           \
        if (threadIdx.x == 0 && blockIdx.x < 4096)                                                 \
            g_abl_wg[4 * blockIdx.x + 3] = ((unsigned long long)__builtin_amdgcn_s_getreg((3 << 11) | 20) << 32) | \
                                           (unsigned)__builtin_amdgcn_s_getreg((31 << 11) | 4);    \
    } while (0)
#else
#define ABL_WG_STAMP(k) \
    do {                \
    } while (0)
#define ABL_WG_IDS() \
    do {             \
    } while (0)
#endif
struct SweepThief {
    uint32_t self, u0, pieces, k;
    uint32_t vic, vn, vs;
    uint64_t ve0, ve1;
    uint32_t tail16;
    bool front, end;
};

__device__ __forceinline__ uint32_t static_iters(uint32_t n, uint32_t tail16, uint32_t ahead)
{
    const uint32_t tail = (uint32_t)(((uint64_t)n * tail16 + 15) / 16);
    return n <= ahead ? n : (n - tail > ahead ? n - tail : ahead);
}

__device__ __forceinline__ unsigned long long thief_issue(const SweepThief &t, unsigned long long *steal)
{
    return __hip_atomic_fetch_add(steal + t.vic, t.front ? 1ull : (1ull << 32), __ATOMIC_RELAXED,
                                  __HIP_MEMORY_SCOPE_AGENT);
}

__device__ __forceinline__ bool thief_take(const SweepThief &t, unsigned long long old, uint32_t qg, uint32_t ahead,
                                           uint64_t &b, uint64_t &e)
{
    (void)ahead;
    const uint32_t f = (uint32_t)old, k = (uint32_t)(old >> 32);
    if ((uint64_t)t.vs + f + k >= t.vn)
        return false;
    const uint32_t it = t.front ? t.vs + f : t.vn - 1 - k;
    b = t.ve0 + (uint64_t)it * qg;
    e = t.ve1;
    return true;
}

__device__ __forceinline__ void thief_next(SweepThief &t, const uint32_t *__restrict__ unit_ent, uint32_t qg,
                                           uint32_t ahead)
{
    t.front = false;
    if (++t.k >= t.pieces) {
        t.end = true;
        return;
    }
    t.vic = t.u0 + (t.self - t.u0 + t.k) % t.pieces;
    t.ve0 = unit_ent[t.vic];
    t.ve1 = unit_ent[t.vic + 1];
    t.vn = (uint32_t)((t.ve1 - t.ve0 + qg - 1) / qg);
    t.vs = static_iters(t.vn, t.tail16, ahead);
}

__device__ bool thief_claim_sync(SweepThief &t, unsigned long long *steal, const uint32_t *__restrict__ unit_ent,
                                 uint32_t qg, uint32_t ahead, uint64_t &b, uint64_t &e)
{
    while (!t.end) {
        if (thief_take(t, thief_issue(t, steal), qg, ahead, b, e))
            return true;
        thief_next(t, unit_ent, qg, ahead);
    }
    return false;
}

template <typename V, int T, typename A, uint32_t J>
__device__ void combine_behind(const uint32_t *__restrict__ panel_row, const uint32_t *__restrict__ panel_unit,
                               const A *__restrict__ cpart, uint32_t stride, V *__restrict__ y,
                               uint32_t *__restrict__ ccount, uint32_t npanels)
{
    constexpr uint32_t kBehindRows = J * T;
    const uint32_t cpp = (stride + kBehindRows - 1) / kBehindRows;
    __shared__ uint32_t claim;
    for (;;) {
        if (threadIdx.x == 0)
            claim = __hip_atomic_fetch_add(ccount, 1u, __ATOMIC_RELAXED, __HIP_MEMORY_SCOPE_AGENT);
        __syncthreads();
        const uint32_t c = claim;
        __syncthreads();
        if (c >= npanels * cpp)
            return;
        const uint32_t p = c / cpp, i0 = (c % cpp) * kBehindRows;
        const uint32_t u0 = panel_unit[p], pieces = panel_unit[p + 1] - u0;
        const uint32_t r0 = panel_row[p], R = panel_row[p + 1] - r0;
        if (pieces < 2 || i0 >= R)
            continue;
        const A *src = cpart + (uint64_t)u0 * stride;
        A acc[J];
#pragma unroll
        for (uint32_t j = 0; j < J; ++j) {
            const uint32_t i = i0 + j * T + threadIdx.x;
            acc[j] = i < R ? src[i] : A(0);
        }
        for (uint32_t t = 1; t < pieces; ++t) {
            const A *sp = src + (uint64_t)t * stride;
#pragma unroll
            for (uint32_t j = 0; j < J; ++j) {
                const uint32_t i = i0 + j * T + threadIdx.x;
                acc[j] += i < R ? sp[i] : A(0);
            }
        }
#pragma unroll
        for (uint32_t j = 0; j < J; ++j) {
            const uint32_t i = i0 + j * T + threadIdx.x;
            if (i < R)
                y[r0 + i] = V(acc[j]);
        }
    }
}

template <typename V, int T, int Q, bool NT, int LAG = 0, int ABL = 0, typename A = double, bool DL = false,
          bool ST = false, typename... FL>
__global__ __launch_bounds__(T) void k_spmv_sweep_packed(
    const uint32_t *__restrict__ rc, const uint32_t *__restrict__ cbase, const V *__restrict__ val,
    const uint32_t *__restrict__ panel_row, const uint32_t *__restrict__ unit_ent,
    const uint32_t *__restrict__ unit_panel, const uint32_t *__restrict__ panel_unit,
    A *__restrict__ part, uint32_t stride, uint32_t *__restrict__ pcnt, const V *__restrict__ x,
    V *__restrict__ y, const uint16_t *__restrict__ row16, const uint8_t *__restrict__ d8,
    const uint32_t *__restrict__ dbase, const uint32_t *__restrict__ side, unsigned long long *__restrict__ steal,
    uint32_t tail16, uint32_t nunits, const A *__restrict__ cpart, uint32_t *__restrict__ ccount,
    uint32_t *__restrict__ cnext, uint32_t npanels, uint32_t cj, FL... fl)
{
    typedef uint32_t u32x2 __attribute__((ext_vector_type(2)));
    typedef uint16_t u16x2 __attribute__((ext_vector_type(2)));
    typedef uint8_t u8x2 __attribute__((ext_vector_type(2)));
    extern __shared__ __attribute__((aligned(16))) unsigned char smem[];
    A *ylds = reinterpret_cast<A *>(smem);
    if (blockIdx.x >= nunits) {
        if (cj == 2)
            combine_behind<V, T, A, 2>(panel_row, panel_unit, cpart, stride, y, ccount, npanels);
        else if (cj == 8)
            combine_behind<V, T, A, 8>(panel_row, panel_unit, cpart, stride, y, ccount, npanels);
        else
            combine_behind<V, T, A, 4>(panel_row, panel_unit, cpart, stride, y, ccount, npanels);
        return;
    }
    if (cnext && blockIdx.x == 0 && threadIdx.x == 0)
        __hip_atomic_store(cnext, 0u, __ATOMIC_RELAXED, __HIP_MEMORY_SCOPE_AGENT);
    const uint32_t p = unit_panel[blockIdx.x];
    const uint32_t pieces = panel_unit[p + 1] - panel_unit[p];
    const uint32_t r0 = panel_row[p], R = panel_row[p + 1] - r0;
    const uint64_t e0 = unit_ent[blockIdx.x], e1 = unit_ent[blockIdx.x + 1];
    __shared__ uint32_t progress[T / 64];
    constexpr uint64_t kGroup = 2ull * T;
    constexpr uint32_t QG = Q * (uint32_t)kGroup, kRing = 8, kAhead = 3;
    static_assert(!ST || (LAG > 0 && LAG < (int)kAhead && kAhead + LAG + 1 <= kRing), "steal ring sizing");
    __shared__ uint32_t ring_b[ST ? kRing : 1], ring_e[ST ? kRing : 1], ring_s[ST ? kRing : 1];
    SweepThief th{blockIdx.x, 0, pieces, 0, blockIdx.x, 0, 0, e0, e1, tail16, true, true};
    ABL_WG_STAMP(0);
    ABL_WG_IDS();
    for (uint32_t i = threadIdx.x; i <= R; i += T)
        ylds[i] = A(0);
    if (threadIdx.x < T / 64)
        progress[threadIdx.x] = 0;
    if constexpr (ST) {
        if (threadIdx.x == 0) {
            th.u0 = panel_unit[p];
            th.vn = (uint32_t)((e1 - e0 + QG - 1) / QG);
            th.vs = static_iters(th.vn, tail16, kAhead);
            th.end = false;
            for (uint32_t t = 0; t < kAhead; ++t) {
                uint64_t b = 0, e = 0;
                bool got = t < th.vs;
                if (got)
                    b = e0 + (uint64_t)t * QG, e = e1;
                else
                    got = thief_claim_sync(th, steal, unit_ent, QG, kAhead, b, e);
                ring_b[t] = got ? (uint32_t)b : 0xFFFFFFFFu;
                ring_e[t] = got ? (uint32_t)e : 0u;
                ring_s[t] = t + 1;
            }
        }
    }
    __syncthreads();
    uint32_t iter = 0;
    A sink = 0;
    const uint32_t wave = __builtin_amdgcn_readfirstlane(threadIdx.x >> 6);
    const uint32_t lane2 = 2u * (threadIdx.x & 63);
    uint64_t base = e0, bound = e1;
    unsigned long long pend = 0;
    bool issued = false;
    for (uint32_t s = 0;; ++s) {
        if constexpr (ST) {
            issued = false;
            if (threadIdx.x == 0 && !th.end && !(th.front && s + kAhead < th.vs)) {
                pend = thief_issue(th, steal);
                issued = true;
            }
            const uint32_t slot = s % kRing;
            uint32_t spin = 0;
            while (__builtin_amdgcn_readfirstlane(__hip_atomic_load(&ring_s[slot], __ATOMIC_ACQUIRE,
                                                                    __HIP_MEMORY_SCOPE_WORKGROUP)) != s + 1 &&
                   ++spin < (1u << 24))
                __builtin_amdgcn_s_sleep(1);
            const uint32_t rb = __builtin_amdgcn_readfirstlane(ring_b[slot]);
            if (rb == 0xFFFFFFFFu || spin >= (1u << 24))
                break;
            base = rb;
            bound = __builtin_amdgcn_readfirstlane(ring_e[slot]);
        } else {
            if (base >= e1)
                break;
        }
        const uint64_t last_chunk = bound > e0 || ST ? bound - 128 : e0;
        u32x2 w[Q];
        uint32_t cb[Q];
        V v[Q][2];
        bool ok[Q];
        u16x2 r16[Q];
        u8x2 dd[Q];
#pragma unroll
        for (int q = 0; q < Q; ++q) {
            uint64_t wbase = base + q * kGroup + 128ull * wave;
            ok[q] = wbase < bound;
            wbase = ok[q] ? wbase : last_chunk;
            if constexpr (ABL == 3 || ABL == 4 || ABL == 9)
                wbase = e0 + ((wbase - e0) & 4095u);
            const uint64_t e = wbase + lane2;
            if constexpr (DL) {
                r16[q] = lds_<NT>(reinterpret_cast<const u16x2 *>(row16 + e));
                dd[q] = lds_<NT>(reinterpret_cast<const u8x2 *>(d8 + e));
                cb[q] = dbase[wbase >> 7];
                loadv<NT, 2>(val, e, v[q]);
                continue;
            }
            if constexpr (ABL == 11) {
                typedef uint16_t u16x2_t __attribute__((ext_vector_type(2)));
                typedef uint8_t u8x2_t __attribute__((ext_vector_type(2)));
                const u16x2_t r16 = lds_<NT>(reinterpret_cast<const u16x2_t *>(reinterpret_cast<const uint16_t *>(rc) + e));
                const u8x2_t d8 = lds_<NT>(reinterpret_cast<const u8x2_t *>(
                    reinterpret_cast<const uint8_t *>(rc) + 2 * (uint64_t)unit_ent[gridDim.x] + e));
                const uint32_t dsum = (uint32_t)(d8.x & 63u) + (uint32_t)(d8.y & 63u);
                uint32_t inc = dsum;
                inc += __builtin_amdgcn_update_dpp(0u, dsum, 0x111, 0xf, 0xf, true);
                inc += __builtin_amdgcn_update_dpp(0u, dsum, 0x112, 0xf, 0xf, true);
                inc += __builtin_amdgcn_update_dpp(0u, dsum, 0x113, 0xf, 0xf, true);
                inc += __builtin_amdgcn_update_dpp(0u, inc, 0x114, 0xf, 0xe, true);
                inc += __builtin_amdgcn_update_dpp(0u, inc, 0x118, 0xf, 0xc, true);
                inc += __builtin_amdgcn_update_dpp(0u, inc, 0x142, 0xa, 0xf, false);
                inc += __builtin_amdgcn_update_dpp(0u, inc, 0x143, 0xc, 0xf, false);
                const uint32_t c0 = inc - dsum + (d8.x & 63u);
                w[q].x = ((uint32_t)(r16.x & 16383u) << 16) | (c0 & 0xFFFFu);
                w[q].y = ((uint32_t)(r16.y & 16383u) << 16) | ((c0 + (d8.y & 63u)) & 0xFFFFu);
            } else {
                w[q] = lds_<NT>(reinterpret_cast<const u32x2 *>(rc + e));
            }
            cb[q] = cbase[wbase >> 7];
            if constexpr (ABL == 10) {
                v[q][0] = v[q][1] = lds_<NT>(val + (wbase >> 1) + (lane2 >> 1));
            } else {
                loadv<NT, 2>(val, e, v[q]);
            }
        }
        V xv[Q][2];
#pragma unroll
        for (int q = 0; q < Q; ++q) {
            if constexpr (DL) {
                uint32_t cx, cy;
                if (cb[q] & 0x80000000u) {
                    const uint64_t sb = (uint64_t)(cb[q] & 0x7FFFFFFFu) * kSweepChunk + lane2;
                    const u32x2 cc = lds_<NT>(reinterpret_cast<const u32x2 *>(side + sb));
                    cx = cc.x;
                    cy = cc.y;
                } else {
                    const uint32_t dx = dd[q].x | ((uint32_t)(r16[q].x >> 15) << 8);
                    const uint32_t dy = dd[q].y | ((uint32_t)(r16[q].y >> 15) << 8);
                    const uint32_t i0 = wave_inclusive_sum(dx), i1 = wave_inclusive_sum(dy);
                    cx = cb[q] + i0;
                    cy = cb[q] + (uint32_t)__builtin_amdgcn_readlane(i0, 63) + i1;
                }
                xv[q][0] = x[cx];
                xv[q][1] = x[cy];
            } else if constexpr (ABL == 2 || ABL == 5) {
                xv[q][0] = V(w[q].x & 1u);
                xv[q][1] = V(w[q].y & 1u);
            } else if constexpr (ABL == 6) {
                xv[q][0] = __builtin_nontemporal_load(x + cb[q] + (w[q].x & 0xFFFFu));
                xv[q][1] = __builtin_nontemporal_load(x + cb[q] + (w[q].y & 0xFFFFu));
            } else if constexpr (ABL == 7) {
                xv[q][0] = __hip_atomic_load(x + cb[q] + (w[q].x & 0xFFFFu), __ATOMIC_RELAXED, __HIP_MEMORY_SCOPE_AGENT);
                xv[q][1] = __hip_atomic_load(x + cb[q] + (w[q].y & 0xFFFFu), __ATOMIC_RELAXED, __HIP_MEMORY_SCOPE_AGENT);
            } else {
                const uint32_t m = (ABL == 1 || ABL == 4 || ABL == 9) ? 0x7FFFu : 0xFFFFFFFFu;
                xv[q][0] = x[(cb[q] + (w[q].x & 0xFFFFu)) & m];
                xv[q][1] = x[(cb[q] + (w[q].y & 0xFFFFu)) & m];
            }
        }
        if constexpr (ABL == 8 || ABL == 9) {
#pragma unroll
            for (int q = 0; q < Q; ++q)
                sink += A(v[q][0]) * A(xv[q][0]) + A(v[q][1]) * A(xv[q][1]);
        } else {
            uint32_t ri[2 * Q];
            A pv[2 * Q];
#pragma unroll
            for (int q = 0; q < Q; ++q) {
                if constexpr (DL) {
                    ri[2 * q] = ok[q] ? (uint32_t)(r16[q].x & 0x7FFFu) : R;
                    ri[2 * q + 1] = ok[q] ? (uint32_t)(r16[q].y & 0x7FFFu) : R;
                } else {
                    ri[2 * q] = ok[q] ? (w[q].x >> 16) : R;
                    ri[2 * q + 1] = ok[q] ? (w[q].y >> 16) : R;
                }
                pv[2 * q] = A(v[q][0]) * A(xv[q][0]);
                pv[2 * q + 1] = A(v[q][1]) * A(xv[q][1]);
            }
            lds_add_n<2 * Q>(ylds, ri, pv);
        }
        if constexpr (ST) {
            if (threadIdx.x == 0) {
                uint64_t b = 0, e = 0;
                bool got = false;
                if (issued) {
                    got = thief_take(th, pend, QG, kAhead, b, e);
                    if (!got) {
                        thief_next(th, unit_ent, QG, kAhead);
                        got = thief_claim_sync(th, steal, unit_ent, QG, kAhead, b, e);
                    }
                } else if (!th.end && th.front && s + kAhead < th.vs) {
                    got = true;
                    b = e0 + (uint64_t)(s + kAhead) * QG;
                    e = e1;
                }
                const uint32_t slot = (s + kAhead) % kRing;
                ring_b[slot] = got ? (uint32_t)b : 0xFFFFFFFFu;
                ring_e[slot] = got ? (uint32_t)e : 0u;
                __hip_atomic_store(&ring_s[slot], s + kAhead + 1, __ATOMIC_RELEASE, __HIP_MEMORY_SCOPE_WORKGROUP);
            }
        } else {
            base += QG;
        }
        if constexpr (LAG == 0) {
            __syncthreads();
        } else {
            ++iter;
            if ((threadIdx.x & 63) == 0)
                __hip_atomic_store(&progress[wave], iter, __ATOMIC_RELAXED, __HIP_MEMORY_SCOPE_WORKGROUP);
            for (;;) {
                const uint32_t lane = threadIdx.x & 63;
                uint32_t pr = lane < T / 64
                                  ? __hip_atomic_load(&progress[lane], __ATOMIC_RELAXED, __HIP_MEMORY_SCOPE_WORKGROUP)
                                  : 0xFFFFFFFFu;
#pragma unroll
                for (int d = 1; d < T / 64; d <<= 1) {
                    const uint32_t o = __shfl_xor(pr, d, 64);
                    pr = o < pr ? o : pr;
                }
                if (__builtin_amdgcn_readfirstlane(pr) + LAG >= iter)
                    break;
                __builtin_amdgcn_s_sleep(1);
            }
        }
    }
    if constexpr (ABL == 8 || ABL == 9)
        lds_add(&ylds[R], sink);
    __syncthreads();
    ABL_WG_STAMP(1);
    if constexpr (sizeof...(FL) == 0) {
        write_panel<V, T, A>(ylds, R, y + r0, pieces, part, stride, panel_unit[p], pcnt ? pcnt + p : nullptr);
    } else {
        const auto args = std::make_tuple(fl...);
        uint32_t *yflag = std::get<0>(args);
        const uint32_t yepoch = std::get<1>(args);
        V *yhost = std::get<2>(args);
        write_panel<V, T, A>(ylds, R, (yhost ? yhost : y) + r0, pieces, part, stride, panel_unit[p],
                             pcnt ? pcnt + p : nullptr);
        asm volatile("s_waitcnt vmcnt(0)" ::: "memory");
        __syncthreads();
        if (threadIdx.x == 0)
            __hip_atomic_store(yflag + p, yepoch, __ATOMIC_RELEASE, __HIP_MEMORY_SCOPE_SYSTEM);
    }
    ABL_WG_STAMP(2);
}


template <typename V, int T, int Q, bool PK, int ORD, typename A = double>
__global__ __launch_bounds__(T) void k_spmv_sweep_turn(
    const uint32_t *__restrict__ col, const uint32_t *__restrict__ cbase, const uint16_t *__restrict__ srow16,
    const V *__restrict__ val, const uint32_t *__restrict__ panel_row, const uint32_t *__restrict__ unit_ent,
    const uint32_t *__restrict__ unit_panel, const uint32_t *__restrict__ panel_unit, A *__restrict__ part,
    uint32_t stride, uint32_t *__restrict__ pcnt, const V *__restrict__ x, V *__restrict__ y)
{
    typedef uint32_t u32x2 __attribute__((ext_vector_type(2)));
    typedef uint16_t u16x2 __attribute__((ext_vector_type(2)));
    constexpr uint32_t W = T / 64;
    extern __shared__ __attribute__((aligned(16))) unsigned char smem[];
    A *ylds = reinterpret_cast<A *>(smem);
    __shared__ uint32_t turn;
    __shared__ uint32_t progress[W];
    const uint32_t p = unit_panel[blockIdx.x];
    const uint32_t pieces = panel_unit[p + 1] - panel_unit[p];
    const uint32_t r0 = panel_row[p], R = panel_row[p + 1] - r0;
    const uint64_t e0 = unit_ent[blockIdx.x], e1 = unit_ent[blockIdx.x + 1];
    for (uint32_t i = threadIdx.x; i <= R; i += T)
        ylds[i] = A(0);
    if (threadIdx.x == 0)
        turn = 0;
    if (threadIdx.x < W)
        progress[threadIdx.x] = 0;
    __syncthreads();
    constexpr uint64_t kGroup = 2ull * T;
    constexpr uint64_t kStep = Q * kGroup;
    const uint32_t wave = __builtin_amdgcn_readfirstlane(threadIdx.x >> 6);
    const uint32_t lane2 = 2u * (threadIdx.x & 63);
    const uint64_t last_chunk = e1 > e0 ? e1 - 128 : e0;
    struct EB {
        u32x2 w[Q];
        uint32_t cb[Q];
        u16x2 r[Q];
        V v[Q][2];
        bool ok[Q];
    };
    struct DB {
        V x[Q][2], v[Q][2];
        uint32_t r[2 * Q];
    };
    auto ld = [&](uint64_t base, EB &e) {
#pragma unroll
        for (int q = 0; q < Q; ++q) {
            uint64_t wbase = base + q * kGroup + 128ull * wave;
            e.ok[q] = wbase < e1;
            wbase = e.ok[q] ? wbase : last_chunk;
            const uint64_t ei = wbase + lane2;
            e.w[q] = lds_<true>(reinterpret_cast<const u32x2 *>(col + ei));
            if constexpr (PK)
                e.cb[q] = cbase[wbase >> 7];
            else
                e.r[q] = lds_<true>(reinterpret_cast<const u16x2 *>(srow16 + ei));
            loadv<true, 2>(val, ei, e.v[q]);
        }
    };
    auto gat = [&](const EB &e, DB &d) {
#pragma unroll
        for (int q = 0; q < Q; ++q) {
            if constexpr (PK) {
                d.x[q][0] = x[e.cb[q] + (e.w[q].x & 0xFFFFu)];
                d.x[q][1] = x[e.cb[q] + (e.w[q].y & 0xFFFFu)];
                d.r[2 * q] = e.ok[q] ? (e.w[q].x >> 16) : R;
                d.r[2 * q + 1] = e.ok[q] ? (e.w[q].y >> 16) : R;
            } else {
                d.x[q][0] = x[e.w[q].x];
                d.x[q][1] = x[e.w[q].y];
                d.r[2 * q] = e.ok[q] ? (uint32_t)e.r[q].x : R;
                d.r[2 * q + 1] = e.ok[q] ? (uint32_t)e.r[q].y : R;
            }
            d.v[q][0] = e.v[q][0];
            d.v[q][1] = e.v[q][1];
        }
    };
    auto step = [&](uint64_t base, uint32_t my, EB &e, const DB &cur, DB &fill) {
        gat(e, fill);
        ld(base + 4 * kStep, e);
        A pv[2 * Q];
#pragma unroll
        for (int q = 0; q < Q; ++q) {
            pv[2 * q] = A(cur.v[q][0]) * A(cur.x[q][0]);
            pv[2 * q + 1] = A(cur.v[q][1]) * A(cur.x[q][1]);
        }
        if constexpr (ORD >= 2) {
            lds_add_n<2 * Q>(ylds, cur.r, pv);
            if constexpr (ORD == 2) {
                const uint32_t iter = my / W + 1;
                if ((threadIdx.x & 63) == 0)
                    __hip_atomic_store(&progress[wave], iter, __ATOMIC_RELAXED, __HIP_MEMORY_SCOPE_WORKGROUP);
                for (;;) {
                    const uint32_t lane = threadIdx.x & 63;
                    uint32_t pr = lane < W ? __hip_atomic_load(&progress[lane], __ATOMIC_RELAXED, __HIP_MEMORY_SCOPE_WORKGROUP)
                                           : 0xFFFFFFFFu;
#pragma unroll
                    for (int d = 1; d < (int)W; d <<= 1) {
                        const uint32_t o = __shfl_xor(pr, d, 64);
                        pr = o < pr ? o : pr;
                    }
                    if (__builtin_amdgcn_readfirstlane(pr) + 2 >= iter)
                        break;
                    __builtin_amdgcn_s_sleep(1);
                }
            }
            return;
        }
        while (__builtin_amdgcn_readfirstlane(__hip_atomic_load(&turn, __ATOMIC_ACQUIRE, __HIP_MEMORY_SCOPE_WORKGROUP)) != my) {
        }
        lds_add_n<2 * Q>(ylds, cur.r, pv);
        if constexpr (ORD == 0) {
            __builtin_amdgcn_s_waitcnt(0xC07F);
            if ((threadIdx.x & 63) == 0)
                __hip_atomic_store(&turn, my + 1, __ATOMIC_RELEASE, __HIP_MEMORY_SCOPE_WORKGROUP);
        } else {
            __atomic_signal_fence(__ATOMIC_SEQ_CST);
            if ((threadIdx.x & 63) == 0)
                __hip_atomic_store(&turn, my + 1, __ATOMIC_RELAXED, __HIP_MEMORY_SCOPE_WORKGROUP);
        }
    };
    const uint32_t nit = (uint32_t)((e1 - e0 + kStep - 1) / kStep);
    if (nit == 0) {
        __syncthreads();
        write_panel<V, T, A>(ylds, R, y + r0, pieces, part, stride, panel_unit[p], pcnt ? pcnt + p : nullptr);
        return;
    }
    EB ea, eb;
    DB d0, d1, d2;
    ld(e0, ea);
    ld(e0 + kStep, eb);
    gat(ea, d0);
    ld(e0 + 2 * kStep, ea);
    gat(eb, d1);
    ld(e0 + 3 * kStep, eb);
    uint32_t my = wave;
    uint64_t base = e0;
    uint32_t it = 0;
#define TSTEP(E, C, F)       \
    step(base, my, E, C, F); \
    base += kStep;           \
    my += W;                 \
    if (++it >= nit)         \
        break;
    while (it < nit) {
        TSTEP(ea, d0, d2)
        TSTEP(eb, d1, d0)
        TSTEP(ea, d2, d1)
        TSTEP(eb, d0, d2)
        TSTEP(ea, d1, d0)
        TSTEP(eb, d2, d1)
    }
#undef TSTEP
    if constexpr (ORD == 2)
        if ((threadIdx.x & 63) == 0)
            __hip_atomic_store(&progress[wave], 0xFFFFFFF0u, __ATOMIC_RELAXED, __HIP_MEMORY_SCOPE_WORKGROUP);
    __syncthreads();
    write_panel<V, T, A>(ylds, R, y + r0, pieces, part, stride, panel_unit[p], pcnt ? pcnt + p : nullptr);
}

__global__ void k_sweep_chunk_base(const uint32_t *__restrict__ col, uint64_t nchunks, uint32_t G,
                                   uint32_t *__restrict__ cbase, uint32_t *__restrict__ bad, uint8_t *__restrict__ wide)
{
    const uint64_t c = (uint64_t)blockIdx.x * blockDim.x + threadIdx.x;
    if (c >= nchunks)
        return;
    uint32_t lo = 0xFFFFFFFFu, hi = 0;
    for (uint32_t k = 0; k < G; ++k) {
        const uint32_t v = col[c * G + k];
        lo = v < lo ? v : lo;
        hi = v > hi ? v : hi;
    }
    cbase[c] = lo;
    wide[c] = hi - lo >= 65536u;
    if (hi - lo >= 65536u)
        atomicAdd(bad, 1u);
}

__global__ void k_sweep_pack_rc(uint32_t *__restrict__ col, const uint16_t *__restrict__ row,
                                const uint32_t *__restrict__ cbase, uint64_t n, uint32_t gshift,
                                const uint8_t *__restrict__ wide)
{
    const uint64_t k = (uint64_t)blockIdx.x * blockDim.x + threadIdx.x;
    if (k >= n)
        return;
    const uint64_t c = k >> gshift;
    col[k] = ((uint32_t)row[k] << 16) | (wide[c] ? 0u : col[k] - cbase[c]);
}

__global__ void k_sweep_lane_order_u32(const uint32_t *__restrict__ in, uint64_t n, uint32_t *__restrict__ out)
{
    const uint64_t k = (uint64_t)blockIdx.x * blockDim.x + threadIdx.x;
    if (k >= n)
        return;
    const uint64_t c = k & ~(uint64_t)127, w = k & 127;
    out[c + 2 * (w & 63) + (w >> 6)] = in[k];
}

template <typename V>
__global__ void k_sweep_lane_order(const uint32_t *__restrict__ rc_in, const V *__restrict__ v_in, uint64_t n,
                                   uint32_t *__restrict__ rc_out, V *__restrict__ v_out)
{
    const uint64_t k = (uint64_t)blockIdx.x * blockDim.x + threadIdx.x;
    if (k >= n)
        return;
    const uint64_t c = k & ~(uint64_t)127, w = k & 127;
    const uint64_t m = c + 2 * (w & 63) + (w >> 6);
    rc_out[m] = rc_in[k];
    v_out[m] = v_in[k];
}

template <typename V>
__global__ void k_sweep_delta(uint32_t *__restrict__ rc, V *__restrict__ val, uint64_t nchunks,
                              uint16_t *__restrict__ row16, uint8_t *__restrict__ d8, uint8_t *__restrict__ flag,
                              const uint8_t *__restrict__ wide)
{
    const uint64_t c = (uint64_t)blockIdx.x * blockDim.x + threadIdx.x;
    if (c >= nchunks)
        return;
    constexpr int G = (int)kSweepChunk;
    uint32_t w[G];
    V v[G];
    uint32_t *cw = rc + c * G;
    V *cv = val + c * G;
    for (int k = 0; k < G; ++k) {
        const int m = 2 * (k & 63) + (k >> 6);
        w[k] = cw[m];
        v[k] = cv[m];
    }
    for (int k = 1; k < G; ++k) {
        const uint32_t wk = w[k];
        const V vk = v[k];
        int j = k - 1;
        while (j >= 0 && (w[j] & 0xFFFFu) > (wk & 0xFFFFu)) {
            w[j + 1] = w[j];
            v[j + 1] = v[j];
            --j;
        }
        w[j + 1] = wk;
        v[j + 1] = vk;
    }
    uint32_t prev = 0;
    bool big = false;
    for (int k = 0; k < G; ++k) {
        const int m = 2 * (k & 63) + (k >> 6);
        const uint32_t off = w[k] & 0xFFFFu;
        const uint32_t d = off - prev;
        big |= d > 511u;
        cw[m] = w[k];
        cv[m] = v[k];
        row16[c * G + m] = (uint16_t)((w[k] >> 16) | ((d >> 8) & 1u) << 15);
        d8[c * G + m] = (uint8_t)d;
        prev = off;
    }
    flag[c] = big || wide[c] ? 1 : 0;
}

__global__ void k_sweep_delta_base(const uint32_t *__restrict__ rc, const uint32_t *__restrict__ cbase,
                                   const uint32_t *__restrict__ sidx, uint64_t nchunks, uint32_t *__restrict__ dbase,
                                   uint32_t *__restrict__ side, const uint8_t *__restrict__ wide,
                                   const uint32_t *__restrict__ abs_col)
{
    const uint64_t c = (uint64_t)blockIdx.x * blockDim.x + threadIdx.x;
    if (c >= nchunks)
        return;
    const uint32_t k = sidx[c];
    if (k == 0xFFFFFFFFu) {
        dbase[c] = cbase[c];
        return;
    }
    dbase[c] = 0x80000000u | k;
    for (uint64_t m = 0; m < kSweepChunk; ++m)
        side[(uint64_t)k * kSweepChunk + m] =
            wide[c] ? abs_col[c * kSweepChunk + m] : cbase[c] + (rc[c * kSweepChunk + m] & 0xFFFFu);
}

__global__ void k_sweep_delta_decode(const uint16_t *__restrict__ row16, const uint8_t *__restrict__ d8,
                                     const uint32_t *__restrict__ dbase, const uint32_t *__restrict__ cbase,
                                     const uint32_t *__restrict__ side, uint64_t nchunks, uint32_t *__restrict__ rc)
{
    const uint64_t c = (uint64_t)blockIdx.x * blockDim.x + threadIdx.x;
    if (c >= nchunks)
        return;
    constexpr int G = (int)kSweepChunk;
    const uint32_t db = dbase[c];
    uint32_t off = 0;
    for (int k = 0; k < G; ++k) {
        const uint64_t m = c * G + 2 * (k & 63) + (k >> 6);
        const uint32_t rw = row16[m];
        if (db & 0x80000000u)
            off = side[(uint64_t)(db & 0x7FFFFFFFu) * G + (m - c * G)] - cbase[c];
        else
            off += (uint32_t)d8[m] | ((rw >> 15) << 8);
        rc[m] = ((rw & 0x7FFFu) << 16) | off;
    }
}

int sweep_materialize_rc(spmv_plan &p)
{
    if (!p.sweep_delta || p.d_s_col || p.ent_pad == 0)
        return 0;
    if (p.sweep_wide) {
        set_error("sweep variant needs the 12-byte entries, which this plan's wide chunks cannot hold");
        return 1;
    }
    const uint64_t nchunks = p.ent_pad / kSweepChunk;
    SPMV_TRY(hipSetDevice(p.device));
    SPMV_TRY(hipMalloc((void **)&p.d_s_col, p.ent_pad * 4));
    hipLaunchKernelGGL(k_sweep_delta_decode, dim3((unsigned)((nchunks + 63) / 64)), dim3(64), 0, nullptr, p.d_s_row16,
                       p.d_s_d8, p.d_s_dbase, p.d_s_cbase, p.d_s_side, nchunks, p.d_s_col);
    SPMV_TRY(hipGetLastError());
    SPMV_TRY(hipDeviceSynchronize());
    return 0;
}

__global__ void k_sweep_keys(const IndexType *__restrict__ rp, const IndexType *__restrict__ col,
                             const uint32_t *__restrict__ panel_row, uint32_t npanels, IndexType nrows,
                             uint64_t nbuckets, uint32_t shift, uint32_t *__restrict__ keys,
                             uint32_t *__restrict__ idx)
{
    const uint64_t r = (uint64_t)blockIdx.x * blockDim.x + threadIdx.x;
    if (r >= nrows)
        return;
    uint32_t lo = 0, hi = npanels;
    while (hi - lo > 1) {
        const uint32_t mid = (lo + hi) / 2;
        if (panel_row[mid] <= r)
            lo = mid;
        else
            hi = mid;
    }
    const uint64_t pbase = (uint64_t)lo * nbuckets;
    for (IndexType j = rp[r]; j < rp[r + 1]; ++j) {
        keys[j] = (uint32_t)(pbase + (col[j] >> shift));
        idx[j] = j;
    }
}

template <typename V>
__global__ void k_sweep_scatter(const uint32_t *__restrict__ keys, const uint32_t *__restrict__ idx,
                                uint64_t nnz, uint64_t nbuckets, const IndexType *__restrict__ rp,
                                IndexType nrows, const IndexType *__restrict__ col_src,
                                const V *__restrict__ val_src, const uint32_t *__restrict__ panel_row,
                                const uint32_t *__restrict__ off, const uint32_t *__restrict__ poff,
                                uint32_t *__restrict__ s_col, uint16_t *__restrict__ s_row,
                                V *__restrict__ s_val)
{
    const uint64_t k = (uint64_t)blockIdx.x * blockDim.x + threadIdx.x;
    if (k >= nnz)
        return;
    const uint32_t p = (uint32_t)(keys[k] / nbuckets);
    const uint32_t j = idx[k];
    uint32_t lo = 0, hi = nrows;
    while (hi - lo > 1) {
        const uint32_t mid = lo + (hi - lo) / 2;
        if (rp[mid] <= j)
            lo = mid;
        else
            hi = mid;
    }
    const uint64_t dst = (uint64_t)poff[p] + (k - off[p]);
    s_col[dst] = col_src[j];
    s_row[dst] = (uint16_t)(lo - panel_row[p]);
    s_val[dst] = val_src[j];
}

template <typename V>
__global__ void k_sweep_pad(uint32_t npanels, const uint32_t *__restrict__ panel_row,
                            const uint32_t *__restrict__ off, const uint32_t *__restrict__ poff,
                            uint32_t *__restrict__ s_col, uint16_t *__restrict__ s_row, V *__restrict__ s_val)
{
    const uint32_t p = blockIdx.x * blockDim.x + threadIdx.x;
    if (p >= npanels)
        return;
    const uint32_t R = panel_row[p + 1] - panel_row[p];
    const uint64_t first_pad = (uint64_t)poff[p] + (off[p + 1] - off[p]);
    const uint32_t pad_col = first_pad > poff[p] ? s_col[first_pad - 1] : 0u;
    for (uint64_t d = first_pad; d < poff[p + 1]; ++d) {
        s_col[d] = pad_col;
        s_row[d] = (uint16_t)R;
        s_val[d] = V(0);
    }
}

__global__ void k_locality(const IndexType *__restrict__ rp, const IndexType *__restrict__ col, IndexType nrows,
                           uint32_t stride, unsigned long long *__restrict__ counts)
{
    const uint64_t r = ((uint64_t)blockIdx.x * blockDim.x + threadIdx.x) * stride;
    if (r >= nrows)
        return;
    const IndexType b = rp[r], e = rp[r + 1];
    if (e - b < 2)
        return;
    const IndexType last = e - b > 65 ? b + 65 : e;
    unsigned long long pairs = 0, near = 0;
    for (IndexType k = b + 1; k < last; ++k) {
        const IndexType c0 = col[k - 1], c1 = col[k];
        const IndexType d = c1 > c0 ? c1 - c0 : c0 - c1;
        ++pairs;
        near += d < 64;
    }
    atomicAdd(&counts[0], pairs);
    atomicAdd(&counts[1], near);
}

template <int T, typename A>
static void launch_sweep_t(const spmv_plan &p, const ValueType *d_x, ValueType *d_y, hipStream_t s, bool warm,
                           void *part_buf, const sweep_behind &bh)
{
    const size_t lds = (size_t(p.panel_rmax) + 1) * sizeof(A);
    const dim3 grid((unsigned)p.nunits), block(T);
    const dim3 gridb((unsigned)p.nunits + (bh.cpart ? bh.blocks : 0u));
    A *part = reinterpret_cast<A *>(part_buf);
    uint32_t *pcnt = p.sweep_split > 1 && p.d_panel_cnt ? p.d_panel_cnt : nullptr;
#define SWEEP(E, Q, SYNC, NT)                                                                     \
    launch_or_warm(warm, k_spmv_sweep<ValueType, T, E, Q, SYNC, NT, A>, grid, block, lds, s, p.d_s_col,   \
                       p.d_s_row, p.d_s_val, p.d_panel_row, p.d_unit_ent, p.d_unit_panel, p.d_panel_unit, part, p.panel_rmax + 1, pcnt, d_x, d_y)
#define TURN(PK, ORD)                                                                              \
    launch_or_warm(warm, k_spmv_sweep_turn<ValueType, T, 2, PK, ORD, A>, grid, block, lds, s, p.d_s_col,          \
                   p.d_s_cbase, p.d_s_row, p.d_s_val, p.d_panel_row, p.d_unit_ent, p.d_unit_panel, p.d_panel_unit, \
                   part, p.panel_rmax + 1, pcnt, d_x, d_y)
#ifdef SPMV_ABLATIONS
    if (p.sweep_packed && p.sweep_variant == 52) {
        TURN(true, 2);
        return;
    }
    if (p.sweep_packed && p.sweep_variant == 51) {
        TURN(true, 3);
        return;
    }
#endif
    if (p.sweep_det || p.sweep_variant == kSweepTurn || p.sweep_variant == kSweepTurnOrdered) {
#ifdef SPMV_ABLATIONS
        if (p.sweep_variant == kSweepTurn) {
            if (p.sweep_packed) TURN(true, 1); else TURN(false, 1);
            return;
        }
#endif
        if (p.sweep_packed) TURN(true, 0); else TURN(false, 0);
        return;
    }
#undef TURN
    if (p.sweep_packed) {
#define PKN(NT, Q, LAG, ABL)                                                                        \
    launch_or_warm(warm, k_spmv_sweep_packed<ValueType, T, Q, NT, LAG, ABL, A>, grid, block, lds, s, p.d_s_col, \
                       p.d_s_cbase, p.d_s_val, p.d_panel_row, p.d_unit_ent, p.d_unit_panel, p.d_panel_unit, part, p.panel_rmax + 1, pcnt, d_x, d_y, \
                       (const uint16_t *)nullptr, (const uint8_t *)nullptr, (const uint32_t *)nullptr, (const uint32_t *)nullptr, \
                       (unsigned long long *)nullptr, 0u, (uint32_t)p.nunits, (const A *)nullptr, (uint32_t *)nullptr, (uint32_t *)nullptr, 0u, 0u)
#define PKD(ST, TAIL)                                                                                 \
    launch_or_warm(warm, k_spmv_sweep_packed<ValueType, T, 2, true, 2, 0, A, true, ST>, gridb, block, lds, s, p.d_s_col, \
                       p.d_s_cbase, p.d_s_val, p.d_panel_row, p.d_unit_ent, p.d_unit_panel, p.d_panel_unit, part, p.panel_rmax + 1, pcnt, d_x, d_y, \
                       p.d_s_row16, p.d_s_d8, p.d_s_dbase, p.d_s_side, ST ? p.d_steal : (unsigned long long *)nullptr, (uint32_t)(TAIL), \
                       (uint32_t)p.nunits, reinterpret_cast<const A *>(bh.cpart), bh.ccount, bh.cnext, (uint32_t)p.npanels, bh.rows_per_thread)
#define PKDF()                                                                                        \
    launch_or_warm(warm, k_spmv_sweep_packed<ValueType, T, 2, true, 2, 0, A, true, false, uint32_t *, uint32_t, ValueType *>, gridb, block, lds, s, \
                   p.d_s_col, p.d_s_cbase, p.d_s_val, p.d_panel_row, p.d_unit_ent, p.d_unit_panel, p.d_panel_unit, part, \
                   p.panel_rmax + 1, pcnt, d_x, d_y, p.d_s_row16, p.d_s_d8, p.d_s_dbase, p.d_s_side,               \
                   (unsigned long long *)nullptr, 0u, (uint32_t)p.nunits, (const A *)nullptr, (uint32_t *)nullptr,  \
                   (uint32_t *)nullptr, (uint32_t)p.npanels, 0u, p.y_flag, p.y_epoch, p.y_host)
#define PKF()                                                                                         \
    launch_or_warm(warm, k_spmv_sweep_packed<ValueType, T, 2, true, 2, 0, A, false, false, uint32_t *, uint32_t, ValueType *>, grid, block, lds, s, p.d_s_col, \
                   p.d_s_cbase, p.d_s_val, p.d_panel_row, p.d_unit_ent, p.d_unit_panel, p.d_panel_unit, part,        \
                   p.panel_rmax + 1, pcnt, d_x, d_y, (const uint16_t *)nullptr, (const uint8_t *)nullptr,           \
                   (const uint32_t *)nullptr, (const uint32_t *)nullptr, (unsigned long long *)nullptr, 0u,          \
                   (uint32_t)p.nunits, (const A *)nullptr, (uint32_t *)nullptr, (uint32_t *)nullptr, 0u, 0u,        \
                   p.y_flag, p.y_epoch, p.y_host)
#define PK(Q, LAG) PKN(true, Q, LAG, 0)
#define PKA(ABL) PKN(true, 2, 2, ABL)
        switch (p.sweep_variant) {
#ifdef SPMV_ABLATIONS
        case 15: PK(2, 0); break;
        case 20: PK(4, 0); break;
        case 22: PK(8, 0); break;
        case 26: PK(4, 1); break;
        case 27: PK(4, 2); break;
        case 29: PK(2, 4); break;
        case 30: PK(2, 1); break;
        case 31: PK(3, 2); break;
        case 32: PK(1, 2); break;
        case 33: PK(1, 4); break;
        case 34: PK(2, 3); break;
        case 35: PK(2, 2); break;
        case 60: if (p.nr_cols >= 32768) { PKA(1); } else { PK(2, 2); } break;
        case 61: PKA(2); break;
        case 62: PKA(3); break;
        case 63: if (p.nr_cols >= 32768) { PKA(4); } else { PK(2, 2); } break;
        case 59: PK(2, 1000); break;
        case 56: PKN(false, 2, 2, 0); break;
        case 54: PKA(8); break;
        case 55: if (p.nr_cols >= 32768) { PKA(9); } else { PK(2, 2); } break;
        case 57: PKA(6); break;
        case 58: PKA(7); break;
        case 53: PKA(10); break;
        case 50: if (p.panel_rmax >= 16384) { PKA(11); } else { PK(2, 2); } break;
#endif
        default:
            if (p.sweep_delta) {
#ifdef SPMV_ABLATIONS
                if (p.sweep_steal && (p.sweep_variant == 37 || p.sweep_variant == 38 || p.sweep_variant == 39)) {
                    PKD(true, p.sweep_variant == 37 ? 8 : p.sweep_variant == 38 ? 16 : 4);
                    break;
                }
#endif
                if (p.y_flag || warm) PKDF();
                if (!p.y_flag) PKD(false, 0);
            } else {
                if (p.y_flag || warm) PKF();
                if (!p.y_flag) PK(2, 2);
            }
            break;
        }
#undef PKD
#undef PKDF
#undef PKF
#undef PKA
#undef PK
#undef PKN
        return;
    }
    switch (p.sweep_variant) {
#ifdef SPMV_ABLATIONS
    case 40: SWEEP(4, 1, false, false); break;
    case 1: SWEEP(4, 1, false, true); break;
    case 3: SWEEP(4, 1, true, true); break;
    case 7: SWEEP(4, 2, true, true); break;
    case 15: SWEEP(2, 2, true, true); break;
    case 22: SWEEP(2, 8, true, true); break;
#endif
    default: SWEEP(2, 4, true, true); break;
    }
#undef SWEEP
}

bool sweep_can_flag_panels(const spmv_plan &p)
{
    if (p.kernel == kKernelBinned)
        return p.npanels > 0 && p.variant != 51 && p.variant != 52;
    return p.kernel == kKernelSweep && p.sweep_packed && !p.sweep_det && p.sweep_split == 1 && p.npanels > 0 &&
           (p.sweep_variant == 0 || p.sweep_variant == 28);
}

bool sweep_behind_ok(const spmv_plan &p)
{
    if (!p.sweep_packed || !p.sweep_delta || p.sweep_det || p.sweep_split < 2 || p.d_panel_cnt)
        return false;
    switch (p.sweep_variant) {
    case 15: case 20: case 22: case 26: case 27: case 29: case 30: case 31: case 32: case 33: case 34:
    case 35: case 37: case 38: case 39: case kSweepTurn: case kSweepTurnOrdered:
        return false;
    default:
        return !(p.sweep_variant >= 50 && p.sweep_variant <= 63);
    }
}

template <typename A>
static void launch_sweep_a(const spmv_plan &p, const ValueType *d_x, ValueType *d_y, hipStream_t s, bool warm,
                           int phase, void *part, const sweep_behind &bh)
{
    if (phase != 2) {
        switch (p.sweep_threads) {
        case 256: launch_sweep_t<256, A>(p, d_x, d_y, s, warm, part, bh); break;
        case 512: launch_sweep_t<512, A>(p, d_x, d_y, s, warm, part, bh); break;
        default: launch_sweep_t<1024, A>(p, d_x, d_y, s, warm, part, bh); break;
        }
    }
    if (phase != 1 && p.sweep_split > 1 && !p.d_panel_cnt) {
        const dim3 grid((p.panel_rmax + 255) / 256, (unsigned)p.npanels);
        launch_or_warm(warm, k_sweep_combine<ValueType, A>, grid, dim3(256), 0, s, p.d_panel_row, p.d_panel_unit,
                       reinterpret_cast<const A *>(part), p.panel_rmax + 1, d_y, p.d_steal);
    }
}

hipError_t launch_sweep(const spmv_plan &p, const ValueType *d_x, ValueType *d_y, hipStream_t s, bool warm, int phase,
                        void *part, const sweep_behind *behind)
{
    if (p.npanels == 0)
        return hipSuccess;
    if (!part)
        part = p.d_part;
    const sweep_behind none{};
    if (behind && (behind->cpart || behind->cnext) && !sweep_behind_ok(p))
        return hipErrorNotSupported;
    const sweep_behind &bh = behind ? *behind : none;
    if constexpr (sizeof(ValueType) == 4) {
        if (p.sweep_acc_bytes == 4) {
            launch_sweep_a<float>(p, d_x, d_y, s, warm, phase, part, bh);
            return hipGetLastError();
        }
    }
    launch_sweep_a<double>(p, d_x, d_y, s, warm, phase, part, bh);
    return hipGetLastError();
}

static const char kWho[] = "build_sweep";

static int sweep_sort_entries(spmv_plan &p, const sweep_units &u, const IndexType *h_rp, const IndexType *d_col_src,
                              const ValueType *d_val_src, hipStream_t s)
{
    const IndexType n = p.nr_rows;
    const uint64_t nnz = p.nnz;
    const uint32_t S = (uint32_t)p.npanels;
    const uint32_t *d_srow = p.d_panel_row;
    uint32_t shift = 0;
    while ((uint64_t(S) * ((uint64_t(p.nr_cols) >> shift) + 1)) >= (1ull << 32))
        ++shift;
    const uint64_t nbuckets = (uint64_t(p.nr_cols) >> shift) + 1;
    int end_bit = 1;
    while (end_bit < 32 && (1ull << end_bit) < uint64_t(S) * nbuckets)
        ++end_bit;
    device_buf<uint32_t> d_off, d_poff, k0, k1, i0, i1;
    device_buf<IndexType> d_rp;
    device_buf<unsigned char> tmp;
    SPMV_BUILD_TRY(d_off.alloc(S + 1));
    SPMV_BUILD_TRY(d_poff.alloc(S + 1));
    SPMV_BUILD_TRY(d_rp.alloc(size_t(n) + 1));
    SPMV_BUILD_TRY(hipMemcpyAsync(d_off, u.off.data(), (S + 1) * 4, hipMemcpyHostToDevice, s));
    SPMV_BUILD_TRY(hipMemcpyAsync(d_poff, u.poff.data(), (S + 1) * 4, hipMemcpyHostToDevice, s));
    SPMV_BUILD_TRY(hipMemcpyAsync(d_rp, h_rp, (size_t(n) + 1) * 4, hipMemcpyHostToDevice, s));
    if (nnz) {
        SPMV_BUILD_TRY(k0.alloc(nnz));
        SPMV_BUILD_TRY(k1.alloc(nnz));
        SPMV_BUILD_TRY(i0.alloc(nnz));
        SPMV_BUILD_TRY(i1.alloc(nnz));
        SPMV_BUILD_TRY(launch_items(k_sweep_keys, n, 256, s, d_rp.get(), d_col_src, d_srow, S, n, nbuckets, shift,
                                    k0.get(), i0.get()));
        size_t tmp_bytes = 0;
        auto sort = [&](void *work) {
            return hipcub::DeviceRadixSort::SortPairs(work, tmp_bytes, k0.get(), k1.get(), i0.get(), i1.get(), nnz, 0,
                                                      end_bit, s);
        };
        SPMV_BUILD_TRY(sort(nullptr));
        SPMV_BUILD_TRY(tmp.alloc(tmp_bytes));
        SPMV_BUILD_TRY(sort(tmp.p));
        SPMV_BUILD_TRY(launch_items(k_sweep_scatter<ValueType>, nnz, 256, s, k1.get(), i1.get(), nnz, nbuckets,
                                    d_rp.get(), n, d_col_src, d_val_src, d_srow, d_off.get(), d_poff.get(), p.d_s_col,
                                    p.d_s_row, p.d_s_val));
    }
    SPMV_BUILD_TRY(launch_items(k_sweep_pad<ValueType>, S, 256, s, S, d_srow, d_off.get(), d_poff.get(), p.d_s_col,
                                p.d_s_row, p.d_s_val));
    SPMV_BUILD_TRY(hipStreamSynchronize(s));
    return 0;
}

static int sweep_chunk_bases(spmv_plan &p, hipStream_t s, device_buf<uint8_t> &d_wide, uint32_t *bad)
{
    const uint64_t nchunks = p.ent_pad / kSweepChunk;
    device_buf<uint32_t> d_bad;
    SPMV_BUILD_TRY(hipMalloc((void **)&p.d_s_cbase, std::max<uint64_t>(nchunks, 1) * 4));
    SPMV_BUILD_TRY(d_bad.alloc(1));
    SPMV_BUILD_TRY(hipMemsetAsync(d_bad, 0, 4, s));
    SPMV_BUILD_TRY(d_wide.alloc(std::max<uint64_t>(nchunks, 1)));
    if (nchunks)
        SPMV_BUILD_TRY(launch_items(k_sweep_chunk_base, nchunks, 256, s, p.d_s_col, nchunks, (uint32_t)kSweepChunk,
                                    p.d_s_cbase, d_bad.get(), d_wide.get()));
    *bad = 0;
    SPMV_BUILD_TRY(hipMemcpyAsync(bad, d_bad, 4, hipMemcpyDeviceToHost, s));
    SPMV_BUILD_TRY(hipStreamSynchronize(s));
    return 0;
}

static int sweep_pack(spmv_plan &p, hipStream_t s, bool wide, bool lane, const device_buf<uint8_t> &d_wide,
                      device_buf<uint32_t> &d_abs)
{
    if (wide) {
        SPMV_BUILD_TRY(d_abs.alloc(p.ent_pad));
        SPMV_BUILD_TRY(launch_items(k_sweep_lane_order_u32, p.ent_pad, 256, s, p.d_s_col, p.ent_pad, d_abs.get()));
        p.sweep_wide = true;
    }
    SPMV_BUILD_TRY(launch_items(k_sweep_pack_rc, p.ent_pad, 256, s, p.d_s_col, p.d_s_row, p.d_s_cbase, p.ent_pad, 7u,
                                d_wide.get()));
    SPMV_BUILD_TRY(hipStreamSynchronize(s));
    SPMV_BUILD_TRY(hipFree(p.d_s_row));
    p.d_s_row = nullptr;
    p.sweep_packed = true;
    if (!lane)
        return 0;
    device_buf<uint32_t> rc2;
    device_buf<ValueType> v2;
    SPMV_BUILD_TRY(rc2.alloc(p.ent_pad));
    SPMV_BUILD_TRY(v2.alloc(p.ent_pad));
    SPMV_BUILD_TRY(launch_items(k_sweep_lane_order<ValueType>, p.ent_pad, 256, s, p.d_s_col, p.d_s_val, p.ent_pad,
                                rc2.get(), v2.get()));
    SPMV_BUILD_TRY(hipStreamSynchronize(s));
    rc2.swap(p.d_s_col);
    v2.swap(p.d_s_val);
    SPMV_BUILD_TRY(rc2.release());
    SPMV_BUILD_TRY(v2.release());
    p.sweep_lane_order = true;
    return 0;
}

static int sweep_delta_encode(spmv_plan &p, hipStream_t s, const device_buf<uint8_t> &d_wide,
                              const device_buf<uint32_t> &d_abs)
{
    const uint64_t nchunks = p.ent_pad / kSweepChunk;
    SPMV_BUILD_TRY(hipMalloc((void **)&p.d_s_row16, p.ent_pad * 2));
    SPMV_BUILD_TRY(hipMalloc((void **)&p.d_s_d8, p.ent_pad));
    SPMV_BUILD_TRY(hipMalloc((void **)&p.d_s_dbase, nchunks * 4));
    std::vector<uint8_t> hf(nchunks);
    {
        device_buf<uint8_t> d_flag;
        SPMV_BUILD_TRY(d_flag.alloc(nchunks));
        SPMV_BUILD_TRY(launch_items(k_sweep_delta<ValueType>, nchunks, 64, s, p.d_s_col, p.d_s_val, nchunks, p.d_s_row16,
                                    p.d_s_d8, d_flag.get(), d_wide.get()));
        SPMV_BUILD_TRY(hipMemcpyAsync(hf.data(), d_flag, nchunks, hipMemcpyDeviceToHost, s));
        SPMV_BUILD_TRY(hipStreamSynchronize(s));
    }
    std::vector<uint32_t> sidx(nchunks, 0xFFFFFFFFu);
    uint64_t ns = 0;
    for (uint64_t c = 0; c < nchunks; ++c)
        if (hf[c])
            sidx[c] = (uint32_t)ns++;
    p.sweep_side_chunks = ns;
    SPMV_BUILD_TRY(hipMalloc((void **)&p.d_s_side, std::max<uint64_t>(ns, 1) * kSweepChunk * 4));
    device_buf<uint32_t> d_sidx;
    SPMV_BUILD_TRY(d_sidx.alloc(nchunks));
    SPMV_BUILD_TRY(hipMemcpyAsync(d_sidx, sidx.data(), nchunks * 4, hipMemcpyHostToDevice, s));
    SPMV_BUILD_TRY(launch_items(k_sweep_delta_base, nchunks, 256, s, p.d_s_col, p.d_s_cbase, d_sidx.get(), nchunks,
                                p.d_s_dbase, p.d_s_side, d_wide.get(), d_abs.get()));
    SPMV_BUILD_TRY(hipStreamSynchronize(s));
    SPMV_BUILD_TRY(d_sidx.release());
    p.sweep_delta = true;
    p.sweep_steal = p.sweep_split > 1 && p.d_steal && !p.d_panel_cnt;
    SPMV_BUILD_TRY(hipFree(p.d_s_col));
    p.d_s_col = nullptr;
    return 0;
}

int build_sweep(spmv_plan &p, const IndexType *h_rp, const IndexType *d_col_src, const ValueType *d_val_src,
                hipStream_t s)
{
    const IndexType n = p.nr_rows;
    const uint64_t lds_bytes = kSweepLdsBytes * p.sweep_threads / 1024 - 256;
    const char *aenv = ablation_env("SPMV_SWEEP_ACC");
    p.sweep_acc_bytes = sizeof(ValueType) == 4 && aenv && std::atoi(aenv) == 32 ? 4 : 8;
    const uint64_t acc = p.sweep_acc_bytes;
    const uint32_t rmax = (uint32_t)std::min<uint64_t>(lds_bytes / acc - 1, 65534);
    const int chip_cus = device_cu_count(p.device);
    panel_options po;
    po.wgs = (uint64_t)chip_cus * (1024 / p.sweep_threads);
    const char *senv = ablation_env("SPMV_SWEEP_SPLIT");
    po.allow_split = !(senv && senv[0] == '0');
    po.force_split = senv && senv[0] == '2';
    po.acc_bytes = acc;
    const char *denv = std::getenv("SPMV_SWEEP_DETERMINISTIC");
    const bool det = denv && denv[0] == '1';
    const char *xbenv = std::getenv("SPMV_SWEEP_XCC_BIAS");
    double xbias_split = xbenv ? std::atof(xbenv) : 0.0;
    po.xbias = xbenv ? std::atof(xbenv) : chip_cus == 256 ? 0.015 : 0.0;
    if (!(po.xbias > -0.5 && po.xbias < 0.5))
        po.xbias = xbias_split = 0.0;
    po.P_first = min_panels(n, rmax);
    if (const char *ke = ablation_env("SPMV_SWEEP_ROUNDS"); ke && std::atoi(ke) > 0 && po.P_first * 2 >= po.wgs)
        po.P_first = std::max<uint64_t>(po.P_first, (uint64_t)std::min(std::atoi(ke), 8) * po.wgs);
    const char *kenv = ablation_env("SPMV_SWEEP_PIECES");
    panel_cut cut;
    sweep_units u;
    if (int rc = plan_panels(kWho, h_rp, n, p.nnz, rmax, po, cut))
        return rc;
    if (int rc = plan_sweep_units(kWho, h_rp, cut.prow, cut.split_mode, po.wgs, kenv ? std::atoi(kenv) : 0,
                                  xbias_split, u))
        return rc;
    const uint32_t P = (uint32_t)(cut.prow.size() - 1), U = u.punit[P];
    p.npanels = P;
    p.panel_rmax = u.rmax_used;
    p.ent_pad = u.poff[P];
    p.sweep_det = det;
    p.xbias_split = u.xbias_split;
    p.sweep_split = u.sweep_split;
    p.nunits = U;
    if (u.sweep_split > 1) {
        SPMV_BUILD_TRY(hipMalloc((void **)&p.d_part, (uint64_t)U * (uint64_t(u.rmax_used) + 1) * acc));
#ifdef SPMV_ABLATIONS
        SPMV_BUILD_TRY(hipMalloc((void **)&p.d_steal, (uint64_t)U * 8));
        SPMV_BUILD_TRY(hipMemsetAsync(p.d_steal, 0, (uint64_t)U * 8, s));
#endif
        const char *cenv = ablation_env("SPMV_SWEEP_COMBINE");
        if (cenv && std::strcmp(cenv, "fused") == 0) {
            SPMV_BUILD_TRY(hipMalloc((void **)&p.d_panel_cnt, std::max<uint64_t>(P, 1) * 4));
            SPMV_BUILD_TRY(hipMemsetAsync(p.d_panel_cnt, 0, std::max<uint64_t>(P, 1) * 4, s));
        }
    }
    const uint64_t ents = std::max<uint64_t>(p.ent_pad, 4);
    SPMV_BUILD_TRY(hipMalloc((void **)&p.d_unit_panel, u.upanel.size() * 4));
    SPMV_BUILD_TRY(hipMalloc((void **)&p.d_panel_unit, u.punit.size() * 4));
    SPMV_BUILD_TRY(hipMalloc((void **)&p.d_panel_row, (P + 1) * 4));
    SPMV_BUILD_TRY(hipMalloc((void **)&p.d_unit_ent, u.uent.size() * 4));
    SPMV_BUILD_TRY(hipMemcpyAsync(p.d_unit_panel, u.upanel.data(), u.upanel.size() * 4, hipMemcpyHostToDevice, s));
    SPMV_BUILD_TRY(hipMemcpyAsync(p.d_panel_unit, u.punit.data(), u.punit.size() * 4, hipMemcpyHostToDevice, s));
    SPMV_BUILD_TRY(hipMemcpyAsync(p.d_panel_row, cut.prow.data(), (P + 1) * 4, hipMemcpyHostToDevice, s));
    SPMV_BUILD_TRY(hipMemcpyAsync(p.d_unit_ent, u.uent.data(), u.uent.size() * 4, hipMemcpyHostToDevice, s));
    SPMV_BUILD_TRY(hipMalloc((void **)&p.d_s_col, ents * 4));
    SPMV_BUILD_TRY(hipMalloc((void **)&p.d_s_row, ents * 2));
    SPMV_BUILD_TRY(hipMalloc((void **)&p.d_s_val, ents * sizeof(ValueType)));

    if (int rc = sweep_sort_entries(p, u, h_rp, d_col_src, d_val_src, s))
        return rc;
    device_buf<uint8_t> d_wide;
    device_buf<uint32_t> d_abs;
    uint32_t bad = 0;
    if (int rc = sweep_chunk_bases(p, s, d_wide, &bad))
        return rc;
    const uint64_t nchunks = p.ent_pad / kSweepChunk;
    const char *env = ablation_env("SPMV_SWEEP_PACKED");
    const bool want = !(env && env[0] == '0');
    const char *lo = ablation_env("SPMV_SWEEP_LANE_ORDER");
    const bool lane = !(lo && lo[0] == '0');
    const char *de = std::getenv("SPMV_SWEEP_DELTA");
    const bool delta = lane && !(de && de[0] == '0') && !det && nchunks && uint64_t(p.nr_cols) < (1ull << 31) &&
                       u.rmax_used < 32768;
    if ((!bad || (delta && uint64_t(bad) * 10 <= nchunks)) && want && p.ent_pad) {
        if (int rc = sweep_pack(p, s, bad != 0, lane, d_wide, d_abs))
            return rc;
        if (delta)
            if (int rc = sweep_delta_encode(p, s, d_wide, d_abs))
                return rc;
    } else {
        SPMV_BUILD_TRY(hipFree(p.d_s_cbase));
        p.d_s_cbase = nullptr;
    }
    SPMV_BUILD_TRY(hipStreamSynchronize(s));
    return 0;
}

int probe_locality(const IndexType *d_rp, const IndexType *d_col, IndexType n, hipStream_t s, double *frac)
{
    *frac = 1.0;
    if (n == 0)
        return 0;
    unsigned long long *d_cnt = nullptr, h[2] = {0, 0};
    SPMV_TRY(hipMalloc((void **)&d_cnt, 16));
    SPMV_TRY(hipMemsetAsync(d_cnt, 0, 16, s));
    const uint32_t stride = std::max<uint32_t>(1, n / 65536);
    const uint64_t threads = (n + stride - 1) / stride;
    hipLaunchKernelGGL(k_locality, dim3((unsigned)((threads + 255) / 256)), dim3(256), 0, s, d_rp, d_col, n, stride,
                       d_cnt);
    SPMV_TRY(hipGetLastError());
    SPMV_TRY(hipMemcpyAsync(h, d_cnt, 16, hipMemcpyDeviceToHost, s));
    SPMV_TRY(hipStreamSynchronize(s));
    SPMV_TRY(hipFree(d_cnt));
    *frac = h[0] ? double(h[1]) / double(h[0]) : 1.0;
    return 0;
}

}

#ifdef SPMV_ABLATIONS
extern "C" int spmv_abl_wg_times(unsigned long long *out, unsigned n)
{
    if (!out || n > 4 * 4096)
        return 1;
    return hipMemcpyFromSymbol(out, HIP_SYMBOL(spmvhw::g_abl_wg), size_t(n) * 8, 0, hipMemcpyDeviceToHost) != hipSuccess;
}
#endif
```

Baseline: 423.6.

## Pack per-unit sweep metadata into records and vectorize partial-slab write/combine

Adds a 32-byte per-unit record (panel, row range, pieces, unit base, entry range) so sweep kernels load one struct instead of chasing unit_panel/panel_unit/panel_row/unit_ent indirections. Partial-sum slabs get an even stride and are written and combined as two-element vectors with nontemporal loads. The combine paths are templated on piece count (2/4/8) for unrolled summation, and combine_behind takes J at runtime. This cuts dependent metadata loads at kernel start and widens slab traffic, in exchange for more template instantiations and a runtime J loop in combine_behind.

Measured after the change: 424.6 (median of 2 runs). About the same (+0.2%).

```diff
diff --git a/spmv-fpga_amd/csrc/layout.cpp b/spmv-fpga_amd/csrc/layout.cpp
--- a/spmv-fpga_amd/csrc/layout.cpp
+++ b/spmv-fpga_amd/csrc/layout.cpp
@@ -123,6 +123,12 @@
     out.xbias_split = split_mode ? xbias_split : 0.0;
     cut_units(poff, punit, out.xbias_split, out.uent);
     out.sweep_split = multi ? std::max<uint32_t>(split, 2) : 1;
+    out.urec.assign(std::max<uint32_t>(punit[P], 1), sweep_unit_rec{});
+    for (uint32_t q = 0; q < P; ++q)
+        for (uint32_t u = punit[q]; u < punit[q + 1]; ++u)
+            out.urec[u] = {q, prow[q], prow[q + 1] - prow[q], punit[q + 1] - punit[q], punit[q], out.uent[u],
+                           out.uent[u + 1], 0u};
+    out.part_stride = (out.rmax_used + 2) & ~1u;
     return 0;
 }
 
diff --git a/spmv-fpga_amd/csrc/plan.cpp b/spmv-fpga_amd/csrc/plan.cpp
--- a/spmv-fpga_amd/csrc/plan.cpp
+++ b/spmv-fpga_amd/csrc/plan.cpp
@@ -675,7 +675,7 @@
     (void)hipDeviceSynchronize();
     for (void *ptr : {(void *)d_col, (void *)d_val, (void *)d_rowend, (void *)d_tile_info,
                       (void *)d_row_id, (void *)d_head, (void *)d_tail, (void *)d_cross, (void *)d_s_col,
-                      (void *)d_s_row, (void *)d_s_val, (void *)d_panel_row, (void *)d_unit_ent, (void *)d_part, (void *)d_gcount, (void *)d_steal, (void *)d_panel_cnt, (void *)d_unit_panel, (void *)d_panel_unit, (void *)d_rp,
+                      (void *)d_s_row, (void *)d_s_val, (void *)d_panel_row, (void *)d_unit_ent, (void *)d_unit_rec, (void *)d_part, (void *)d_gcount, (void *)d_steal, (void *)d_panel_cnt, (void *)d_unit_panel, (void *)d_panel_unit, (void *)d_rp,
                       (void *)d_s_cbase, (void *)d_s_row16, (void *)d_s_d8, (void *)d_s_dbase, (void *)d_s_side, d_colnar, (void *)d_tile_cbase, (void *)d_kptr, (void *)d_kpos,
                       (void *)d_rp2, (void *)d_rl, (void *)d_chunk_row, (void *)d_bpart, (void *)d_slot_off,
                       (void *)d_sbase, (void *)d_slice_len, (void *)d_b_val, (void *)d_b_colw, (void *)d_b_rowp,
@@ -711,7 +711,7 @@
     if (kernel == kKernelSweep)
         return ent_pad * ((d_s_col ? sizeof(uint32_t) : 0) + (sweep_packed ? 0 : sizeof(uint16_t)) + sizeof(ValueType)) +
                (npanels + 1) * 4 + (nunits + 1) * 4 + (sweep_packed ? ent_pad / kSweepChunk * 4 : 0) +
-               (sweep_split > 1 ? nunits * (uint64_t(panel_rmax) + 1) * sweep_acc_bytes : 0) + nunits * 4 + (npanels + 1) * 4 +
+               (sweep_split > 1 ? nunits * uint64_t(part_stride) * sweep_acc_bytes : 0) + nunits * (4 + sizeof(sweep_unit_rec)) + (npanels + 1) * 4 +
                (d_panel_cnt ? npanels * 4 : 0) +
                (sweep_delta ? ent_pad * 3 + ent_pad / kSweepChunk * 4 + sweep_side_chunks * kSweepChunk * 4 : 0);
     return nnz_pad * (tile_col_bytes + sizeof(ValueType)) + nnz_pad / 8 + (ntiles + 1) * 4 +
@@ -848,7 +848,7 @@
 {
     if (p->gpart.empty()) {
         void *b = nullptr;
-        SPMV_TRY(hipMalloc(&b, p->nunits * (uint64_t(p->panel_rmax) + 1) * p->sweep_acc_bytes));
+        SPMV_TRY(hipMalloc(&b, p->nunits * uint64_t(p->part_stride) * p->sweep_acc_bytes));
         p->gpart.push_back(b);
     }
     return 0;
diff --git a/spmv-fpga_amd/csrc/spmv_host.hpp b/spmv-fpga_amd/csrc/spmv_host.hpp
--- a/spmv-fpga_amd/csrc/spmv_host.hpp
+++ b/spmv-fpga_amd/csrc/spmv_host.hpp
@@ -62,12 +62,24 @@
 int plan_panels(const char *who, const IndexType *h_rp, IndexType n, uint64_t nnz, uint32_t rmax,
                 const panel_options &o, panel_cut &out);
 
+struct alignas(32) sweep_unit_rec {
+    uint32_t panel;
+    uint32_t row0, rows;
+    uint32_t pieces;
+    uint32_t unit0;
+    uint32_t ent0, ent1;
+    uint32_t pad;
+};
+static_assert(sizeof(sweep_unit_rec) == 32, "one record per 32 bytes");
+
 struct sweep_units {
     std::vector<uint32_t> off, poff;
     std::vector<uint32_t> punit;
     std::vector<uint32_t> upanel;
     std::vector<uint32_t> uent;
+    std::vector<sweep_unit_rec> urec;
     uint32_t rmax_used = 0;
+    uint32_t part_stride = 2;
     uint32_t sweep_split = 1;
     double xbias_split = 0.0;
 };
diff --git a/spmv-fpga_amd/csrc/spmv_internal.hpp b/spmv-fpga_amd/csrc/spmv_internal.hpp
--- a/spmv-fpga_amd/csrc/spmv_internal.hpp
+++ b/spmv-fpga_amd/csrc/spmv_internal.hpp
@@ -100,6 +100,8 @@
     uint32_t sweep_split = 1;
     uint32_t *d_unit_panel = nullptr;
     uint32_t *d_panel_unit = nullptr;
+    spmvhw::sweep_unit_rec *d_unit_rec = nullptr;
+    uint32_t part_stride = 2;
     void *d_part = nullptr;
     std::vector<void *> gpart;
     uint32_t *d_gcount = nullptr;
diff --git a/spmv-fpga_amd/csrc/sweep.hip b/spmv-fpga_amd/csrc/sweep.hip
--- a/spmv-fpga_amd/csrc/sweep.hip
+++ b/spmv-fpga_amd/csrc/sweep.hip
@@ -103,6 +103,34 @@
     }
 }
 
+#ifdef SPMV_ABLATIONS
+__device__ int g_abl_slab_form;
+#endif
+template <typename T>
+struct Pair {
+    typedef T type __attribute__((ext_vector_type(2)));
+};
+
+template <typename A>
+__device__ __forceinline__ void slab_store(typename Pair<A>::type *p, typename Pair<A>::type v)
+{
+#ifdef SPMV_ABLATIONS
+    const int form = g_abl_slab_form & 3;
+    if (form == 1) {
+        __builtin_nontemporal_store(v, p);
+        return;
+    }
+    if (form == 2) {
+        A *q = reinterpret_cast<A *>(p);
+        const A v0 = v.x, v1 = v.y;
+        __hip_atomic_store(q, v0, __ATOMIC_RELAXED, __HIP_MEMORY_SCOPE_AGENT);
+        __hip_atomic_store(q + 1, v1, __ATOMIC_RELAXED, __HIP_MEMORY_SCOPE_AGENT);
+        return;
+    }
+#endif
+    *p = v;
+}
+
 template <typename V, int T, typename A>
 __device__ __forceinline__ void write_panel(const A *__restrict__ ylds, uint32_t R, V *__restrict__ y,
                                             uint32_t pieces, A *__restrict__ part, uint32_t stride,
@@ -114,8 +142,20 @@
         return;
     }
     A *dst = part + (uint64_t)blockIdx.x * stride;
-    for (uint32_t i = threadIdx.x; i < R; i += T)
-        dst[i] = ylds[i];
+    bool pairs = true;
+#ifdef SPMV_ABLATIONS
+    pairs = !(g_abl_slab_form & 16);
+#endif
+    if (pairs) {
+        typedef typename Pair<A>::type a2;
+        const a2 *src2 = reinterpret_cast<const a2 *>(ylds);
+        a2 *dst2 = reinterpret_cast<a2 *>(dst);
+        for (uint32_t i = threadIdx.x; 2 * i < R; i += T)
+            slab_store<A>(dst2 + i, src2[i]);
+    } else {
+        for (uint32_t i = threadIdx.x; i < R; i += T)
+            dst[i] = ylds[i];
+    }
     if (!pcnt)
         return;
     __shared__ uint32_t last;
@@ -144,7 +184,79 @@
         __hip_atomic_store(pcnt, 0u, __ATOMIC_RELAXED, __HIP_MEMORY_SCOPE_AGENT);
 }
 
-template <typename V, typename A>
+template <typename A>
+__device__ __forceinline__ typename Pair<A>::type load_part(const A *__restrict__ p)
+{
+    typedef typename Pair<A>::type A2;
+#ifdef SPMV_ABLATIONS
+    if (g_abl_slab_form & 4)
+        return *reinterpret_cast<const A2 *>(p);
+#endif
+    return __builtin_nontemporal_load(reinterpret_cast<const A2 *>(p));
+}
+
+template <typename A, int NP, int G>
+__device__ __forceinline__ void sum_pieces(const A *__restrict__ src, uint32_t stride, uint32_t pieces,
+                                           const uint32_t (&i)[G], typename Pair<A>::type (&acc)[G])
+{
+    typedef typename Pair<A>::type A2;
+    if constexpr (NP > 0) {
+        A2 v[G][NP];
+#pragma unroll
+        for (int g = 0; g < G; ++g)
+#pragma unroll
+            for (int t = 0; t < NP; ++t)
+                v[g][t] = load_part(src + (uint64_t)t * stride + i[g]);
+#pragma unroll
+        for (int g = 0; g < G; ++g) {
+            acc[g] = v[g][0];
+#pragma unroll
+            for (int t = 1; t < NP; ++t)
+                acc[g] += v[g][t];
+        }
+    } else {
+#pragma unroll
+        for (int g = 0; g < G; ++g)
+            acc[g] = load_part(src + i[g]);
+        for (uint32_t t = 1; t < pieces; ++t) {
+            const A *sp = src + (uint64_t)t * stride;
+#pragma unroll
+            for (int g = 0; g < G; ++g)
+                acc[g] += load_part(sp + i[g]);
+        }
+    }
+}
+
+template <typename A, int G>
+__device__ __forceinline__ void sum_pieces_any(const A *__restrict__ src, uint32_t stride, uint32_t pieces,
+                                               const uint32_t (&i)[G], typename Pair<A>::type (&acc)[G])
+{
+    switch (pieces) {
+    case 2: sum_pieces<A, 2, G>(src, stride, pieces, i, acc); break;
+    case 4: sum_pieces<A, 4, G>(src, stride, pieces, i, acc); break;
+    case 8: sum_pieces<A, 8, G>(src, stride, pieces, i, acc); break;
+    default: sum_pieces<A, 0, G>(src, stride, pieces, i, acc); break;
+    }
+}
+
+
+template <typename V, typename A2>
+__device__ __forceinline__ void store_pair(V *__restrict__ y, A2 acc, bool two)
+{
+    typedef typename Pair<V>::type V2;
+    if (two && (reinterpret_cast<uintptr_t>(y) & (sizeof(V2) - 1)) == 0) {
+        V2 o;
+        o.x = V(acc.x);
+        o.y = V(acc.y);
+        *reinterpret_cast<V2 *>(y) = o;
+        return;
+    }
+    y[0] = V(acc.x);
+    if (two)
+        y[1] = V(acc.y);
+}
+
+template <typename V, typename A, int NP>
 __global__ __launch_bounds__(256) void k_sweep_combine(const uint32_t *__restrict__ panel_row,
                                                        const uint32_t *__restrict__ panel_unit,
                                                        const A *__restrict__ part, uint32_t stride,
@@ -156,14 +268,17 @@
         for (uint32_t t = threadIdx.x; t < u1 - u0; t += 256)
             steal[u0 + t] = 0;
     const uint32_t r0 = panel_row[p], R = panel_row[p + 1] - r0;
-    const uint32_t i = blockIdx.x * 256 + threadIdx.x;
+    const uint32_t i = 2 * (blockIdx.x * 256 + threadIdx.x);
     if (u1 - u0 < 2 || i >= R)
         return;
-    const A *src = part + (uint64_t)u0 * stride + i;
-    A acc = src[0];
-    for (uint32_t t = 1; t < u1 - u0; ++t)
-        acc += src[(uint64_t)t * stride];
-    y[r0 + i] = V(acc);
+    const A *src = part + (uint64_t)u0 * stride;
+    const uint32_t ii[1] = {i};
+    typename Pair<A>::type acc[1];
+    if (NP > 0 && u1 - u0 == NP)
+        sum_pieces<A, NP, 1>(src, stride, NP, ii, acc);
+    else
+        sum_pieces<A, 0, 1>(src, stride, u1 - u0, ii, acc);
+    store_pair(y + r0 + i, acc[0], i + 1 < R);
 }
 
 template <typename V, int T, int E, int Q, bool SYNC, bool NT, typename A = double>
@@ -299,12 +414,12 @@
     return false;
 }
 
-template <typename V, int T, typename A, uint32_t J>
+template <typename V, int T, typename A>
 __device__ void combine_behind(const uint32_t *__restrict__ panel_row, const uint32_t *__restrict__ panel_unit,
                                const A *__restrict__ cpart, uint32_t stride, V *__restrict__ y,
-                               uint32_t *__restrict__ ccount, uint32_t npanels)
-{
-    constexpr uint32_t kBehindRows = J * T;
+                               uint32_t *__restrict__ ccount, uint32_t npanels, uint32_t J)
+{
+    const uint32_t kBehindRows = J * T;
     const uint32_t cpp = (stride + kBehindRows - 1) / kBehindRows;
     __shared__ uint32_t claim;
     for (;;) {
@@ -321,25 +436,45 @@
         if (pieces < 2 || i0 >= R)
             continue;
         const A *src = cpart + (uint64_t)u0 * stride;
-        A acc[J];
-#pragma unroll
-        for (uint32_t j = 0; j < J; ++j) {
-            const uint32_t i = i0 + j * T + threadIdx.x;
-            acc[j] = i < R ? src[i] : A(0);
-        }
-        for (uint32_t t = 1; t < pieces; ++t) {
-            const A *sp = src + (uint64_t)t * stride;
-#pragma unroll
-            for (uint32_t j = 0; j < J; ++j) {
+#ifdef SPMV_ABLATIONS
+        if ((g_abl_slab_form & 8) && J == 4) {
+            A acc[4];
+#pragma unroll
+            for (uint32_t j = 0; j < 4; ++j) {
                 const uint32_t i = i0 + j * T + threadIdx.x;
-                acc[j] += i < R ? sp[i] : A(0);
+                acc[j] = i < R ? src[i] : A(0);
             }
-        }
-#pragma unroll
-        for (uint32_t j = 0; j < J; ++j) {
-            const uint32_t i = i0 + j * T + threadIdx.x;
-            if (i < R)
-                y[r0 + i] = V(acc[j]);
+            for (uint32_t t = 1; t < pieces; ++t) {
+                const A *sp = src + (uint64_t)t * stride;
+#pragma unroll
+                for (uint32_t j = 0; j < 4; ++j) {
+                    const uint32_t i = i0 + j * T + threadIdx.x;
+                    acc[j] += i < R ? sp[i] : A(0);
+                }
+            }
+#pragma unroll
+            for (uint32_t j = 0; j < 4; ++j) {
+                const uint32_t i = i0 + j * T + threadIdx.x;
+                if (i < R)
+                    y[r0 + i] = V(acc[j]);
+            }
+            continue;
+        }
+#endif
+        constexpr int G = 2;
+        for (uint32_t j = 0; j < J / 2; j += G) {
+            uint32_t i[G], ic[G];
+            typename Pair<A>::type acc[G];
+#pragma unroll
+            for (int g = 0; g < G; ++g) {
+                i[g] = j + g < J / 2 ? i0 + 2 * ((j + g) * T + threadIdx.x) : R;
+                ic[g] = i[g] < R ? i[g] : 0;
+            }
+            sum_pieces_any<A, G>(src, stride, pieces, ic, acc);
+#pragma unroll
+            for (int g = 0; g < G; ++g)
+                if (i[g] < R)
+                    store_pair(y + r0 + i[g], acc[g], i[g] + 1 < R);
         }
     }
 }
@@ -349,7 +484,7 @@
 __global__ __launch_bounds__(T) void k_spmv_sweep_packed(
     const uint32_t *__restrict__ rc, const uint32_t *__restrict__ cbase, const V *__restrict__ val,
     const uint32_t *__restrict__ panel_row, const uint32_t *__restrict__ unit_ent,
-    const uint32_t *__restrict__ unit_panel, const uint32_t *__restrict__ panel_unit,
+    const sweep_unit_rec *__restrict__ units, const uint32_t *__restrict__ panel_unit,
     A *__restrict__ part, uint32_t stride, uint32_t *__restrict__ pcnt, const V *__restrict__ x,
     V *__restrict__ y, const uint16_t *__restrict__ row16, const uint8_t *__restrict__ d8,
     const uint32_t *__restrict__ dbase, const uint32_t *__restrict__ side, unsigned long long *__restrict__ steal,
@@ -362,20 +497,16 @@
     extern __shared__ __attribute__((aligned(16))) unsigned char smem[];
     A *ylds = reinterpret_cast<A *>(smem);
     if (blockIdx.x >= nunits) {
-        if (cj == 2)
-            combine_behind<V, T, A, 2>(panel_row, panel_unit, cpart, stride, y, ccount, npanels);
-        else if (cj == 8)
-            combine_behind<V, T, A, 8>(panel_row, panel_unit, cpart, stride, y, ccount, npanels);
-        else
-            combine_behind<V, T, A, 4>(panel_row, panel_unit, cpart, stride, y, ccount, npanels);
+        combine_behind<V, T, A>(panel_row, panel_unit, cpart, stride, y, ccount, npanels,
+                                cj == 2 || cj == 8 ? cj : 4u);
         return;
     }
     if (cnext && blockIdx.x == 0 && threadIdx.x == 0)
         __hip_atomic_store(cnext, 0u, __ATOMIC_RELAXED, __HIP_MEMORY_SCOPE_AGENT);
-    const uint32_t p = unit_panel[blockIdx.x];
-    const uint32_t pieces = panel_unit[p + 1] - panel_unit[p];
-    const uint32_t r0 = panel_row[p], R = panel_row[p + 1] - r0;
-    const uint64_t e0 = unit_ent[blockIdx.x], e1 = unit_ent[blockIdx.x + 1];
+    const sweep_unit_rec unit = units[blockIdx.x];
+    const uint32_t p = unit.panel, pieces = unit.pieces;
+    const uint32_t r0 = unit.row0, R = unit.rows;
+    const uint64_t e0 = unit.ent0, e1 = unit.ent1;
     __shared__ uint32_t progress[T / 64];
     constexpr uint64_t kGroup = 2ull * T;
     constexpr uint32_t QG = Q * (uint32_t)kGroup, kRing = 8, kAhead = 3;
@@ -390,7 +521,7 @@
         progress[threadIdx.x] = 0;
     if constexpr (ST) {
         if (threadIdx.x == 0) {
-            th.u0 = panel_unit[p];
+            th.u0 = unit.unit0;
             th.vn = (uint32_t)((e1 - e0 + QG - 1) / QG);
             th.vs = static_iters(th.vn, tail16, kAhead);
             th.end = false;
@@ -592,13 +723,13 @@
     __syncthreads();
     ABL_WG_STAMP(1);
     if constexpr (sizeof...(FL) == 0) {
-        write_panel<V, T, A>(ylds, R, y + r0, pieces, part, stride, panel_unit[p], pcnt ? pcnt + p : nullptr);
+        write_panel<V, T, A>(ylds, R, y + r0, pieces, part, stride, unit.unit0, pcnt ? pcnt + p : nullptr);
     } else {
         const auto args = std::make_tuple(fl...);
         uint32_t *yflag = std::get<0>(args);
         const uint32_t yepoch = std::get<1>(args);
         V *yhost = std::get<2>(args);
-        write_panel<V, T, A>(ylds, R, (yhost ? yhost : y) + r0, pieces, part, stride, panel_unit[p],
+        write_panel<V, T, A>(ylds, R, (yhost ? yhost : y) + r0, pieces, part, stride, unit.unit0,
                              pcnt ? pcnt + p : nullptr);
         asm volatile("s_waitcnt vmcnt(0)" ::: "memory");
         __syncthreads();
@@ -613,7 +744,7 @@
 __global__ __launch_bounds__(T) void k_spmv_sweep_turn(
     const uint32_t *__restrict__ col, const uint32_t *__restrict__ cbase, const uint16_t *__restrict__ srow16,
     const V *__restrict__ val, const uint32_t *__restrict__ panel_row, const uint32_t *__restrict__ unit_ent,
-    const uint32_t *__restrict__ unit_panel, const uint32_t *__restrict__ panel_unit, A *__restrict__ part,
+    const sweep_unit_rec *__restrict__ units, const uint32_t *__restrict__ panel_unit, A *__restrict__ part,
     uint32_t stride, uint32_t *__restrict__ pcnt, const V *__restrict__ x, V *__restrict__ y)
 {
     typedef uint32_t u32x2 __attribute__((ext_vector_type(2)));
@@ -623,10 +754,10 @@
     A *ylds = reinterpret_cast<A *>(smem);
     __shared__ uint32_t turn;
     __shared__ uint32_t progress[W];
-    const uint32_t p = unit_panel[blockIdx.x];
-    const uint32_t pieces = panel_unit[p + 1] - panel_unit[p];
-    const uint32_t r0 = panel_row[p], R = panel_row[p + 1] - r0;
-    const uint64_t e0 = unit_ent[blockIdx.x], e1 = unit_ent[blockIdx.x + 1];
+    const sweep_unit_rec unit = units[blockIdx.x];
+    const uint32_t p = unit.panel, pieces = unit.pieces;
+    const uint32_t r0 = unit.row0, R = unit.rows;
+    const uint64_t e0 = unit.ent0, e1 = unit.ent1;
     for (uint32_t i = threadIdx.x; i <= R; i += T)
         ylds[i] = A(0);
     if (threadIdx.x == 0)
@@ -730,7 +861,7 @@
     const uint32_t nit = (uint32_t)((e1 - e0 + kStep - 1) / kStep);
     if (nit == 0) {
         __syncthreads();
-        write_panel<V, T, A>(ylds, R, y + r0, pieces, part, stride, panel_unit[p], pcnt ? pcnt + p : nullptr);
+        write_panel<V, T, A>(ylds, R, y + r0, pieces, part, stride, unit.unit0, pcnt ? pcnt + p : nullptr);
         return;
     }
     EB ea, eb;
@@ -763,7 +894,7 @@
         if ((threadIdx.x & 63) == 0)
             __hip_atomic_store(&progress[wave], 0xFFFFFFF0u, __ATOMIC_RELAXED, __HIP_MEMORY_SCOPE_WORKGROUP);
     __syncthreads();
-    write_panel<V, T, A>(ylds, R, y + r0, pieces, part, stride, panel_unit[p], pcnt ? pcnt + p : nullptr);
+    write_panel<V, T, A>(ylds, R, y + r0, pieces, part, stride, unit.unit0, pcnt ? pcnt + p : nullptr);
 }
 
 __global__ void k_sweep_chunk_base(const uint32_t *__restrict__ col, uint64_t nchunks, uint32_t G,
@@ -1022,11 +1153,11 @@
     uint32_t *pcnt = p.sweep_split > 1 && p.d_panel_cnt ? p.d_panel_cnt : nullptr;
 #define SWEEP(E, Q, SYNC, NT)                                                                     \
     launch_or_warm(warm, k_spmv_sweep<ValueType, T, E, Q, SYNC, NT, A>, grid, block, lds, s, p.d_s_col,   \
-                       p.d_s_row, p.d_s_val, p.d_panel_row, p.d_unit_ent, p.d_unit_panel, p.d_panel_unit, part, p.panel_rmax + 1, pcnt, d_x, d_y)
+                       p.d_s_row, p.d_s_val, p.d_panel_row, p.d_unit_ent, p.d_unit_panel, p.d_panel_unit, part, p.part_stride, pcnt, d_x, d_y)
 #define TURN(PK, ORD)                                                                              \
     launch_or_warm(warm, k_spmv_sweep_turn<ValueType, T, 2, PK, ORD, A>, grid, block, lds, s, p.d_s_col,          \
-                   p.d_s_cbase, p.d_s_row, p.d_s_val, p.d_panel_row, p.d_unit_ent, p.d_unit_panel, p.d_panel_unit, \
-                   part, p.panel_rmax + 1, pcnt, d_x, d_y)
+                   p.d_s_cbase, p.d_s_row, p.d_s_val, p.d_panel_row, p.d_unit_ent, p.d_unit_rec, p.d_panel_unit, \
+                   part, p.part_stride, pcnt, d_x, d_y)
 #ifdef SPMV_ABLATIONS
     if (p.sweep_packed && p.sweep_variant == 52) {
         TURN(true, 2);
@@ -1051,24 +1182,24 @@
     if (p.sweep_packed) {
 #define PKN(NT, Q, LAG, ABL)                                                                        \
     launch_or_warm(warm, k_spmv_sweep_packed<ValueType, T, Q, NT, LAG, ABL, A>, grid, block, lds, s, p.d_s_col, \
-                       p.d_s_cbase, p.d_s_val, p.d_panel_row, p.d_unit_ent, p.d_unit_panel, p.d_panel_unit, part, p.panel_rmax + 1, pcnt, d_x, d_y, \
+                       p.d_s_cbase, p.d_s_val, p.d_panel_row, p.d_unit_ent, p.d_unit_rec, p.d_panel_unit, part, p.part_stride, pcnt, d_x, d_y, \
                        (const uint16_t *)nullptr, (const uint8_t *)nullptr, (const uint32_t *)nullptr, (const uint32_t *)nullptr, \
                        (unsigned long long *)nullptr, 0u, (uint32_t)p.nunits, (const A *)nullptr, (uint32_t *)nullptr, (uint32_t *)nullptr, 0u, 0u)
 #define PKD(ST, TAIL)                                                                                 \
     launch_or_warm(warm, k_spmv_sweep_packed<ValueType, T, 2, true, 2, 0, A, true, ST>, gridb, block, lds, s, p.d_s_col, \
-                       p.d_s_cbase, p.d_s_val, p.d_panel_row, p.d_unit_ent, p.d_unit_panel, p.d_panel_unit, part, p.panel_rmax + 1, pcnt, d_x, d_y, \
+                       p.d_s_cbase, p.d_s_val, p.d_panel_row, p.d_unit_ent, p.d_unit_rec, p.d_panel_unit, part, p.part_stride, pcnt, d_x, d_y, \
                        p.d_s_row16, p.d_s_d8, p.d_s_dbase, p.d_s_side, ST ? p.d_steal : (unsigned long long *)nullptr, (uint32_t)(TAIL), \
                        (uint32_t)p.nunits, reinterpret_cast<const A *>(bh.cpart), bh.ccount, bh.cnext, (uint32_t)p.npanels, bh.rows_per_thread)
 #define PKDF()                                                                                        \
     launch_or_warm(warm, k_spmv_sweep_packed<ValueType, T, 2, true, 2, 0, A, true, false, uint32_t *, uint32_t, ValueType *>, gridb, block, lds, s, \
-                   p.d_s_col, p.d_s_cbase, p.d_s_val, p.d_panel_row, p.d_unit_ent, p.d_unit_panel, p.d_panel_unit, part, \
-                   p.panel_rmax + 1, pcnt, d_x, d_y, p.d_s_row16, p.d_s_d8, p.d_s_dbase, p.d_s_side,               \
+                   p.d_s_col, p.d_s_cbase, p.d_s_val, p.d_panel_row, p.d_unit_ent, p.d_unit_rec, p.d_panel_unit, part, \
+                   p.part_stride, pcnt, d_x, d_y, p.d_s_row16, p.d_s_d8, p.d_s_dbase, p.d_s_side,               \
                    (unsigned long long *)nullptr, 0u, (uint32_t)p.nunits, (const A *)nullptr, (uint32_t *)nullptr,  \
                    (uint32_t *)nullptr, (uint32_t)p.npanels, 0u, p.y_flag, p.y_epoch, p.y_host)
 #define PKF()                                                                                         \
     launch_or_warm(warm, k_spmv_sweep_packed<ValueType, T, 2, true, 2, 0, A, false, false, uint32_t *, uint32_t, ValueType *>, grid, block, lds, s, p.d_s_col, \
-                   p.d_s_cbase, p.d_s_val, p.d_panel_row, p.d_unit_ent, p.d_unit_panel, p.d_panel_unit, part,        \
-                   p.panel_rmax + 1, pcnt, d_x, d_y, (const uint16_t *)nullptr, (const uint8_t *)nullptr,           \
+                   p.d_s_cbase, p.d_s_val, p.d_panel_row, p.d_unit_ent, p.d_unit_rec, p.d_panel_unit, part,        \
+                   p.part_stride, pcnt, d_x, d_y, (const uint16_t *)nullptr, (const uint8_t *)nullptr,           \
                    (const uint32_t *)nullptr, (const uint32_t *)nullptr, (unsigned long long *)nullptr, 0u,          \
                    (uint32_t)p.nunits, (const A *)nullptr, (uint32_t *)nullptr, (uint32_t *)nullptr, 0u, 0u,        \
                    p.y_flag, p.y_epoch, p.y_host)
@@ -1172,9 +1303,17 @@
         }
     }
     if (phase != 1 && p.sweep_split > 1 && !p.d_panel_cnt) {
-        const dim3 grid((p.panel_rmax + 255) / 256, (unsigned)p.npanels);
-        launch_or_warm(warm, k_sweep_combine<ValueType, A>, grid, dim3(256), 0, s, p.d_panel_row, p.d_panel_unit,
-                       reinterpret_cast<const A *>(part), p.panel_rmax + 1, d_y, p.d_steal);
+        const dim3 grid(((p.panel_rmax + 1) / 2 + 255) / 256, (unsigned)p.npanels);
+#define COMBINE(NP)                                                                                                \
+    launch_or_warm(warm, k_sweep_combine<ValueType, A, NP>, grid, dim3(256), 0, s, p.d_panel_row, p.d_panel_unit, \
+                   reinterpret_cast<const A *>(part), p.part_stride, d_y, p.d_steal)
+        switch (p.sweep_split) {
+        case 2: COMBINE(2); break;
+        case 4: COMBINE(4); break;
+        case 8: COMBINE(8); break;
+        default: COMBINE(0); break;
+        }
+#undef COMBINE
     }
 }
 
@@ -1376,8 +1515,9 @@
     p.xbias_split = u.xbias_split;
     p.sweep_split = u.sweep_split;
     p.nunits = U;
+    p.part_stride = u.part_stride;
     if (u.sweep_split > 1) {
-        SPMV_BUILD_TRY(hipMalloc((void **)&p.d_part, (uint64_t)U * (uint64_t(u.rmax_used) + 1) * acc));
+        SPMV_BUILD_TRY(hipMalloc((void **)&p.d_part, (uint64_t)U * uint64_t(u.part_stride) * acc));
 #ifdef SPMV_ABLATIONS
         SPMV_BUILD_TRY(hipMalloc((void **)&p.d_steal, (uint64_t)U * 8));
         SPMV_BUILD_TRY(hipMemsetAsync(p.d_steal, 0, (uint64_t)U * 8, s));
@@ -1397,6 +1537,9 @@
     SPMV_BUILD_TRY(hipMemcpyAsync(p.d_panel_unit, u.punit.data(), u.punit.size() * 4, hipMemcpyHostToDevice, s));
     SPMV_BUILD_TRY(hipMemcpyAsync(p.d_panel_row, cut.prow.data(), (P + 1) * 4, hipMemcpyHostToDevice, s));
     SPMV_BUILD_TRY(hipMemcpyAsync(p.d_unit_ent, u.uent.data(), u.uent.size() * 4, hipMemcpyHostToDevice, s));
+    SPMV_BUILD_TRY(hipMalloc((void **)&p.d_unit_rec, u.urec.size() * sizeof(sweep_unit_rec)));
+    SPMV_BUILD_TRY(hipMemcpyAsync(p.d_unit_rec, u.urec.data(), u.urec.size() * sizeof(sweep_unit_rec),
+                                  hipMemcpyHostToDevice, s));
     SPMV_BUILD_TRY(hipMalloc((void **)&p.d_s_col, ents * 4));
     SPMV_BUILD_TRY(hipMalloc((void **)&p.d_s_row, ents * 2));
     SPMV_BUILD_TRY(hipMalloc((void **)&p.d_s_val, ents * sizeof(ValueType)));
@@ -1459,4 +1602,12 @@
         return 1;
     return hipMemcpyFromSymbol(out, HIP_SYMBOL(spmvhw::g_abl_wg), size_t(n) * 8, 0, hipMemcpyDeviceToHost) != hipSuccess;
 }
+
+extern "C" int spmv_abl_slab_store(int form)
+{
+    if (form < 0 || form > 31 || (form & 3) == 3)
+        return 1;
+    return hipMemcpyToSymbol(HIP_SYMBOL(spmvhw::g_abl_slab_form), &form, sizeof(form), 0, hipMemcpyHostToDevice) !=
+           hipSuccess;
+}
 #endif
```
